# jeya-maria-jose/Medical-Transformer

Hardware: AMD Instinct MI355X
Metric: training images/sec (MedT, 3x128x128) (higher is better)
Workload: dtype f32; 1 GPU; MedT imgsize=128 bs=4/GPU train step (fwd+CE+bwd+Adam), BASELINE.json configs[2] (per GPU: also configs[3]'s shard); global_batch=4, parallelism=dp1

## Files before the change

### include/medt_abi.h

```cpp
#ifndef MEDT_ABI_H
#define MEDT_ABI_H

#include <stddef.h>
#include <stdint.h>

#ifdef __cplusplus
extern "C" {
#endif

#define MEDT_ABI_VERSION 11

#define MEDT_OK            0
#define MEDT_EINVAL       -1
#define MEDT_EUNSUPPORTED -2
#define MEDT_ELAUNCH      -3
#define MEDT_EWORKSPACE   -4

int         medt_abi_version(void);
const char* medt_last_error(void);

void*  medt_queue_create(void);
int    medt_queue_destroy(void* queue);
int    medt_queue_bind(void* queue, void* stream);
size_t medt_queue_pending(const void* queue);
int    medt_queue_flush(void* queue, void* stream);
int    medt_queue_flush2(void* queue, void* stream, void* aux_stream);
int    medt_queue_discard(void* queue);

typedef struct medt_axial_desc {
    int32_t N, C, H, W;
    int32_t G;
    int32_t axis;
    int32_t has_pos;
    int32_t stride;
    int32_t training;
    int32_t bn_groups;
    float   eps;
    float   momentum;
    int32_t out_relu;
    int32_t gate_mode;
    int32_t act_dtype;
} medt_axial_desc;

typedef struct medt_bn_ptrs {
    const float* weight;
    const float* bias;
    float*       running_mean;
    float*       running_var;
    int64_t*     num_batches_tracked;
} medt_bn_ptrs;

typedef struct medt_axial_params {
    const float* w_qkv;
    medt_bn_ptrs bn_qkv;
    medt_bn_ptrs bn_similarity;
    medt_bn_ptrs bn_output;
    const float* relative;
    const float* f_qr;
    const float* f_kr;
    const float* f_sve;
    const float* f_sv;
} medt_axial_params;

typedef struct medt_axial_saved {
    void*  qkv_raw;
    void*  stacked;
    float* lse;
    float* stats;
} medt_axial_saved;

typedef struct medt_axial_grads {
    float* w_qkv;
    float* bn_qkv_weight;  float* bn_qkv_bias;
    float* bn_sim_weight;  float* bn_sim_bias;
    float* bn_out_weight;  float* bn_out_bias;
    float* relative;
    float* gates;
} medt_axial_grads;

size_t medt_axial_stats_floats(const medt_axial_desc*);
size_t medt_axial_workspace_bytes(const medt_axial_desc*);

int medt_axial_layer_fwd(const medt_axial_desc*, const medt_axial_params*, const float* x, float* y,
                         const medt_axial_saved*, void* workspace, size_t workspace_bytes, void* stream);

int medt_axial_layer_bwd(const medt_axial_desc*, const medt_axial_params*, const float* x, const float* y,
                         const float* dy, const medt_axial_saved*, float* dx, const medt_axial_grads*,
                         void* workspace, size_t workspace_bytes, void* stream);

int medt_axial_core_stats(const medt_axial_desc*, const medt_axial_params*, const medt_axial_saved*,
                          void* workspace, size_t workspace_bytes, void* stream);
int medt_axial_core_fwd(const medt_axial_desc*, const medt_axial_params*, const medt_axial_saved*,
                        void* workspace, size_t workspace_bytes, void* stream);
int medt_axial_core_bwd(const medt_axial_desc*, const medt_axial_params*, const medt_axial_saved*, const float* dy,
                        void* workspace, size_t workspace_bytes, void* stream);

typedef struct medt_block_desc {
    int32_t N, C, width, H, W;
    int32_t G;
    int32_t training, bn_groups;
    float   eps, momentum;
} medt_block_desc;

typedef struct medt_block_params {
    const float*      w_down;
    medt_bn_ptrs      bn1;
    medt_axial_params height;
    medt_axial_params width;
    const float*      w_up;
    medt_bn_ptrs      bn2;
} medt_block_params;

typedef struct medt_block_saved {
    float* z1;
    float* y1;
    float* stats1;
    medt_axial_saved height;
    float* y_h;
    medt_axial_saved width;
    float* y_w;
    float* z2;
    float* stats2;
} medt_block_saved;

size_t medt_wopos_block_workspace_bytes(const medt_block_desc*);
int medt_wopos_block_fwd(const medt_block_desc*, const medt_block_params*, const float* x, float* y,
                         const medt_block_saved*, void* workspace, size_t workspace_bytes, void* stream);

typedef struct medt_block_s2_params {
    medt_block_params blk;
    const float*      w_ds;
    medt_bn_ptrs      bn_ds;
} medt_block_s2_params;
typedef struct medt_block_s2_saved {
    medt_block_saved blk;
    float *zd, *yd, *statsd;
} medt_block_s2_saved;
size_t medt_wopos_block_s2_workspace_bytes(const medt_block_desc*);
int medt_wopos_block_s2_fwd(const medt_block_desc*, const medt_block_s2_params*, const float* x, float* y,
                            const medt_block_s2_saved*, void* workspace, size_t workspace_bytes, void* stream);

typedef struct medt_block_grads {
    float *w_down, *bn1_weight, *bn1_bias;
    medt_axial_grads height, width;
    float *w_up, *bn2_weight, *bn2_bias;
} medt_block_grads;
size_t medt_wopos_block_bwd_workspace_bytes(const medt_block_desc*);
int medt_wopos_block_bwd(const medt_block_desc*, const medt_block_params*, const float* x, const float* y, const float* dy,
                         const medt_block_saved*, float* dx, const float* dx_add, const medt_block_grads*,
                         void* workspace, size_t workspace_bytes, void* stream);

typedef struct medt_conv_desc {
    int32_t N, Cin, H, W, Cout;
    int32_t K, stride, pad;
    int32_t has_bias;
    int32_t has_bn;
    int32_t has_res;
    int32_t relu;
    int32_t training, bn_groups;
    float   eps, momentum;
    int32_t lean;
} medt_conv_desc;

size_t medt_conv_stats_floats(const medt_conv_desc*);
size_t medt_conv_workspace_bytes(const medt_conv_desc*);

int medt_conv_block_fwd(const medt_conv_desc*, const float* x, const float* w, const float* bias,
                        const medt_bn_ptrs* bn, const float* res, float* z, float* y, float* stats,
                        void* workspace, size_t workspace_bytes, void* stream);
int medt_conv_block_bwd(const medt_conv_desc*, const float* x, const float* w, const medt_bn_ptrs* bn,
                        const float* z, const float* y, const float* stats, const float* dy,
                        float* dx, float* dw, float* dbias, float* dbn_weight, float* dbn_bias, float* dres,
                        const float* dx_add, void* workspace, size_t workspace_bytes, void* stream);

int medt_gate_mlp_fwd(const float* x, const float* w1, const float* b1, const float* w2, const float* b2, float* xn, float* h,
                      float* o, float* gates, int N, int C, int H, int W, int axis, void* stream);
int medt_gate_mlp_bwd(const float* dgates, const float* gates, const float* o, const float* h, const float* xn,
                      const float* w1, const float* w2, float* scratch, float* dw1, float* db1, float* dw2, float* db2,
                      float* dx, int N, int C, int H, int W, int axis, void* stream);

int medt_up2x_relu_add_fwd(const float* x, const float* skip, float* y, int NC, int H, int W, void* stream);
int medt_up2x_relu_bwd(const float* x, const float* dy, float* dx, int NC, int H, int W, void* stream);

int medt_patch_gather(const float* x, float* xp, int N, int C, int S, int P, int G, void* stream);
int medt_logo_merge_fwd(const float* x, const float* yp, float* y, int N, int C, int S, int P, int G, void* stream);
int medt_logo_merge_bwd(const float* dy, float* dx, float* dyp, int N, int C, int S, int P, int G, void* stream);

size_t medt_ce_partials(int N, int HW);
int medt_ce_fwd(const float* logits, const int64_t* target, float* partials, float* loss_out, int N, int K, int HW,
                int ignore_index, void* stream);
int medt_ce_bwd(const float* logits, const int64_t* target, const float* loss_out, const float* dloss, float* dlogits,
                int N, int K, int HW, int ignore_index, void* stream);

size_t medt_seg_loss_workspace(int N, int K, int HW);
size_t medt_seg_loss_out_floats(int N, int K);
int medt_seg_loss_fwd(const float* logits, const int64_t* target, const float* class_weight, float* partials, float* out,
                      int N, int K, int HW, int ignore_index, float ce_scale, float dice_scale, float eps, void* stream);
int medt_seg_loss_bwd(const float* logits, const int64_t* target, const float* class_weight, const float* out,
                      const float* dloss, float* dlogits, int N, int K, int HW, int ignore_index, float ce_scale,
                      float dice_scale, float eps, void* stream);

int medt_adam_step(float* p, const float* g, float* m, float* v, float* state, size_t n, float lr, float beta1,
                   float beta2, float eps, float weight_decay, float gscale, void* stream);

int medt_relu_mask(const float* a, const float* y, float* out, size_t n, void* stream);

int medt_seg_counts(const float* logits, const int64_t* target, int32_t* counts, int N, int K, int HW, float threshold,
                    void* stream);

int medt_window_gather(const float* image, float* windows, const int32_t* oy, const int32_t* ox, int C, int H, int W, int S,
                       int ny, int nx, void* stream);
int medt_window_blend(const float* win_logits, float* blended, uint8_t* mask, const int32_t* oy, const int32_t* ox, int K,
                      int H, int W, int S, int ny, int nx, float threshold, void* stream);

size_t medt_augment_param_floats(void);
size_t medt_augment_workspace(int N, int th, int tw);
int medt_augment_stats(const uint8_t* image, const float* params, float* workspace, int N, int H, int W, int C, int th,
                       int tw, void* stream);
int medt_augment_apply(const uint8_t* image, const uint8_t* mask, const float* params, float* workspace, float* out_image,
                       int64_t* out_mask, int N, int H, int W, int C, int th, int tw, int use_stats, void* stream);

#define MEDT_EDT_NONE    2147483647
#define MEDT_EDT_MAX_DIM 4096
int medt_edt_cols(const uint8_t* mask, int32_t* g2, int N, int H, int W, int border_mode, void* stream);
int medt_edt_rows(const int32_t* g2, const uint8_t* select, int32_t* d2, int N, int H, int W, void* stream);

int medt_signed_edt(const int64_t* target, int32_t* g2, int32_t* sd2, int N, int H, int W, int fg, int ignore_index, void* stream);
size_t medt_boundary_workspace(int N, int HW);
size_t medt_boundary_out_floats(int N);
int medt_boundary_fwd(const float* logits, const int64_t* target, const int32_t* sd2, const float* alpha, const float* base,
                      float* partials, float* out, int N, int K, int HW, int fg, int ignore_index, void* stream);
int medt_boundary_bwd(const float* logits, const int64_t* target, const int32_t* sd2, const float* out, const float* dloss,
                      float* dlogits, int N, int K, int HW, int fg, int ignore_index, int accumulate, void* stream);

int medt_object_edt2(const int32_t* labels, int32_t* scratch, int32_t* d1sq, int32_t* d2sq, int N, int H, int W, void* stream);
size_t medt_border_workspace(int N, int HW);
size_t medt_border_out_floats(int N);
int medt_border_fwd(const float* logits, const int64_t* target, const int32_t* d1sq, const int32_t* d2sq, float sigma,
                    const float* w0, const float* base, float* partials, float* out, int N, int K, int HW, int fg,
                    int ignore_index, void* stream);
int medt_border_bwd(const float* logits, const int64_t* target, const int32_t* d1sq, const int32_t* d2sq, float sigma,
                    const float* out, const float* dloss, float* dlogits, int N, int K, int HW, int fg, int ignore_index,
                    int accumulate, void* stream);

#define MEDT_LABEL_TILE_H  16
#define MEDT_LABEL_TILE_W  64
#define MEDT_LABEL_MAX_DIM 4096
size_t medt_label_workspace_bytes(int N, int H, int W);
int medt_label_components(const uint8_t* mask, int32_t* labels, int32_t* count, void* workspace, size_t workspace_bytes, int N,
                          int H, int W, int connectivity, int background, void* stream);
int medt_label_tables(const int32_t* labels, int32_t* area, uint8_t* frame, int N, int H, int W, int stride, int max_count,
                      void* stream);
int medt_label_select(const int32_t* labels, const uint8_t* keep, const uint8_t* mask, uint8_t* out, int N, int H, int W,
                      int stride, void* stream);

#define MEDT_PAIR_JOB_INTS 16
int medt_label_boxes(const int32_t* labels, int32_t* box, int N, int H, int W, int stride, int max_count, void* stream);
int medt_pair_hausdorff(const int32_t* la, const int32_t* lb, const int32_t* jobs, int32_t* scratch, int32_t* out, int n_jobs,
                        int col_blocks, int row_blocks, size_t scratch_elems, int n_out, int clear_out, int N, int H, int W,
                        void* stream);

#ifdef __cplusplus
}
#endif
#endif
```

### medical-transformer_amd/csrc/conv.hip

```cpp
#include "defer.h"
#include <type_traits>

namespace medt {

template <int K, int OT>
__global__ __launch_bounds__(MEDT_THREADS) void conv2d_fwd_kernel(
    const float* __restrict__ x, const float* __restrict__ w, const float* __restrict__ bias, float* __restrict__ y,
    float* __restrict__ partials, int Cin, int H, int W, int Cout, int Ho, int Wo, int stride, int pad, int relu,
    int npg, int y_bf16) {
    constexpr int KK = K * K;
    MEDT_STATIC_SHARED float red[MEDT_WAVES * OT * 2 * 2];
    const int HoWo = Ho * Wo, per_group = npg * HoWo, ppg = (per_group + MEDT_THREADS - 1) / MEDT_THREADS;
    const int grp = blockIdx.x / ppg, part = blockIdx.x - grp * ppg, o0 = blockIdx.y * OT;
    const int q = part * MEDT_THREADS + threadIdx.x;
    const bool ok = q < per_group;
    const int ni = ok ? q / HoWo : 0, p = ok ? q - ni * HoWo : 0;
    const int n = grp * npg + ni;
    const int ho = p / Wo, wo = p - ho * Wo;
    const int h0 = ho * stride - pad, w0 = wo * stride - pad;
    float acc[OT];
#pragma unroll
    for (int o = 0; o < OT; ++o) acc[o] = bias ? bias[o0 + o] : 0.f;
    const float* xn = x + (size_t)n * Cin * H * W;
    int off[KK];
#pragma unroll
    for (int kh = 0; kh < K; ++kh)
#pragma unroll
        for (int kw = 0; kw < K; ++kw) {
            const int h = h0 + kh, ww = w0 + kw;
            off[kh * K + kw] = (ok && (unsigned)h < (unsigned)H && (unsigned)ww < (unsigned)W) ? h * W + ww : -1;
        }
    const int HWi = H * W;
    constexpr int U = K == 1 ? 8 : (K == 3 ? 4 : 1);
    auto taps = [&](auto u_tag, int c) {
        constexpr int UU = decltype(u_tag)::value;
        float xr[UU][KK];
#pragma unroll
        for (int u = 0; u < UU; ++u)
#pragma unroll
            for (int t = 0; t < KK; ++t) xr[u][t] = xn[(size_t)(c + u) * HWi + max(off[t], 0)];
        MEDT_SCHED_FENCE();
#pragma unroll
        for (int u = 0; u < UU; ++u) {
            float xv[KK];
#pragma unroll
            for (int t = 0; t < KK; ++t) xv[t] = off[t] >= 0 ? xr[u][t] : 0.f;
#pragma unroll
            for (int o = 0; o < OT; ++o) {
                const float* wp = w + ((size_t)(o0 + o) * Cin + c + u) * KK;
#pragma unroll
                for (int t = 0; t < KK; ++t) acc[o] = fmaf(wp[t], xv[t], acc[o]);
            }
        }
        MEDT_SCHED_FENCE();
    };
    int c = 0;
    for (; c + U <= Cin; c += U) taps(std::integral_constant<int, U>{}, c);
    for (; c < Cin; ++c) taps(std::integral_constant<int, 1>{}, c);
    if (ok) {
        const size_t yo = ((size_t)n * Cout + o0) * HoWo + p;
#pragma unroll
        for (int o = 0; o < OT; ++o) st_act(y, yo + (size_t)o * HoWo, relu ? fmaxf(acc[o], 0.f) : acc[o], y_bf16);
    }
    if (partials) {
        float v[2 * OT];
#pragma unroll
        for (int o = 0; o < OT; ++o) {
            const float a = ok ? acc[o] : 0.f;
            v[2 * o] = a;
            v[2 * o + 1] = a * a;
        }
        block_sum_d<2 * OT>(v, red, reinterpret_cast<double*>(partials) + ((size_t)blockIdx.x * Cout + o0) * 2);
    }
}

int conv2d_parts_per_group(int N, int groups, int HoWo) { return cdiv((N / groups) * HoWo, MEDT_THREADS); }

static int pick_tile(int C, int max_tile, long position_blocks) {
    int t = max_tile;
    while (t > 1 && (C % t != 0 || position_blocks * (C / t) < 512)) t >>= 1;
    while (C % t != 0) t >>= 1;
    return t;
}

template <int K>
static int conv2d_fwd_k(const float* x, const float* w, const float* bias, float* y, float* partials, int N, int Cin,
                        int H, int W, int Cout, int Ho, int Wo, int stride, int pad, int relu, int groups,
                        hipStream_t s, int y_bf16) {
    const int npg = N / groups;
    const unsigned gx = (unsigned)(groups * conv2d_parts_per_group(N, groups, Ho * Wo));
#define MEDT_LAUNCH_FWD(OT)                                                                                        \
    hipLaunchKernelGGL((conv2d_fwd_kernel<K, OT>), dim3(gx, Cout / OT), dim3(MEDT_THREADS), 0, s, x, w, bias, y, partials, \
                       Cin, H, W, Cout, Ho, Wo, stride, pad, relu, npg, y_bf16)
    switch (pick_tile(Cout, K == 7 ? 8 : 16, gx)) {
        case 16: if constexpr (K != 7) { MEDT_LAUNCH_FWD(16); } break;
        case 8: MEDT_LAUNCH_FWD(8); break;
        case 4: MEDT_LAUNCH_FWD(4); break;
        case 2: MEDT_LAUNCH_FWD(2); break;
        default: MEDT_LAUNCH_FWD(1); break;
    }
#undef MEDT_LAUNCH_FWD
    return launch_status("conv2d_fwd");
}

static int conv_thin_mode() {
    static const int m = [] { const char* e = getenv("MEDT_CONV_THIN"); return e ? atoi(e) : 3; }();
    return m;
}
int conv_parts_per_group(int N, int groups, int HoWo, int Cin, int Cout, int K, int stride, int H, int W, int pad) {
    if (H > 0 && (conv_thin_mode() & 1) && !conv_use_mfma(Cin, Cout, K, stride, (long)N * HoWo) && conv_thin_ok(N, groups, Cin, H, W, Cout, K, stride, pad))
        return conv_thin_parts_per_group(N, groups, Cin, H, W, Cout, K, stride, pad);
    if (conv_fwd_ws_ok(Cin, Cout, K, stride, (long)N * HoWo)) return cdiv((N / groups) * HoWo, 64);
    if (!conv_use_mfma(Cin, Cout, K, stride, (long)N * HoWo)) return conv2d_parts_per_group(N, groups, HoWo);
    if (conv_mfma_scratch_floats(N, groups, HoWo, Cin, Cout, K, H > 0 && conv_rows16_ok(Cin, H, W, K, stride, pad)) > 0) return conv2d_parts_per_group(N, groups, HoWo);
    return conv_mfma_parts_per_group(N, groups, HoWo);
}

size_t conv2d_fwd_scratch_floats(int N, int groups, int Cin, int H, int W, int Cout, int K, int stride, int pad) {
    const int Ho = (H + 2 * pad - K) / stride + 1, Wo = (W + 2 * pad - K) / stride + 1;
    if (!conv_use_mfma(Cin, Cout, K, stride, (long)N * Ho * Wo)) return 0;
    return conv_mfma_scratch_floats(N, groups, Ho * Wo, Cin, Cout, K, conv_rows16_ok(Cin, H, W, K, stride, pad));
}

size_t conv2d_bwd_data_scratch_floats(int N, int Cin, int H, int W, int Cout, int K, int stride, int pad) {
    if (stride != 1 || K - 1 - pad < 0 || !conv_use_mfma(Cout, Cin, K, 1, (long)N * H * W)) return 0;
    return conv_mfma_scratch_floats(N, 1, H * W, Cout, Cin, K, conv_rows16_ok(Cout, H, W, K, 1, K - 1 - pad));
}

template <int K, int OT>
__global__ __launch_bounds__(MEDT_THREADS) void conv2d_fwd_ws_kernel(
    const float* __restrict__ x, const float* __restrict__ w, const float* __restrict__ bias, float* __restrict__ y,
    float* __restrict__ partials, int Cin, int H, int W, int Cout, int Ho, int Wo, int stride, int pad, int relu,
    int npg, int y_bf16) {
    constexpr int KK = K * K;
    MEDT_STATIC_SHARED float red[3][OT][64];
    extern __shared__ __attribute__((aligned(16))) float wl[];
    const int lane = threadIdx.x & 63, wv = __builtin_amdgcn_readfirstlane(threadIdx.x >> 6);
    const int HoWo = Ho * Wo, per_group = npg * HoWo, ppg = (per_group + 63) / 64;
    const int grp = blockIdx.x / ppg, part = blockIdx.x - grp * ppg, o0 = blockIdx.y * OT;
    {
        const int nw = OT * Cin * KK;
        const float* src = w + (size_t)o0 * Cin * KK;
        for (int e0 = threadIdx.x; e0 < nw; e0 += 8 * MEDT_THREADS) {
            float v[8];
#pragma unroll
            for (int u = 0; u < 8; ++u) v[u] = src[min(e0 + u * MEDT_THREADS, nw - 1)];
            MEDT_SCHED_FENCE();
#pragma unroll
            for (int u = 0; u < 8; ++u)
                if (e0 + u * MEDT_THREADS < nw) wl[e0 + u * MEDT_THREADS] = v[u];
        }
    }
    const int q = part * 64 + lane;
    const bool ok = q < per_group;
    const int ni = ok ? q / HoWo : 0, p = ok ? q - ni * HoWo : 0;
    const int n = grp * npg + ni;
    const int ho = p / Wo, wo = p - ho * Wo;
    const int h0 = ho * stride - pad, w0 = wo * stride - pad;
    int off[KK];
#pragma unroll
    for (int kh = 0; kh < K; ++kh)
#pragma unroll
        for (int kw = 0; kw < K; ++kw) {
            const int h = h0 + kh, ww = w0 + kw;
            off[kh * K + kw] = (ok && (unsigned)h < (unsigned)H && (unsigned)ww < (unsigned)W) ? h * W + ww : -1;
        }
    float acc[OT];
#pragma unroll
    for (int o = 0; o < OT; ++o) acc[o] = 0.f;
    const float* xn = x + (size_t)n * Cin * H * W;
    const int HWi = H * W;
    const int cb = (Cin * wv) / 4, ce = (Cin * (wv + 1)) / 4;
    __syncthreads();
    constexpr int U = K == 1 ? 16 : 4;
    auto taps = [&](auto u_tag, int c) {
        constexpr int UU = decltype(u_tag)::value;
        float xr[UU][KK];
#pragma unroll
        for (int u = 0; u < UU; ++u)
#pragma unroll
            for (int t = 0; t < KK; ++t) xr[u][t] = xn[(size_t)(c + u) * HWi + max(off[t], 0)];
        MEDT_SCHED_FENCE();
#pragma unroll
        for (int u = 0; u < UU; ++u) {
            float xv[KK];
#pragma unroll
            for (int t = 0; t < KK; ++t) xv[t] = off[t] >= 0 ? xr[u][t] : 0.f;
#pragma unroll
            for (int o = 0; o < OT; ++o) {
                const float* wp = wl + (o * Cin + c + u) * KK;
#pragma unroll
                for (int t = 0; t < KK; ++t) acc[o] = fmaf(wp[t], xv[t], acc[o]);
            }
        }
        MEDT_SCHED_FENCE();
    };
    int c = cb;
    for (; c + U <= ce; c += U) taps(std::integral_constant<int, U>{}, c);
    for (; c < ce; ++c) taps(std::integral_constant<int, 1>{}, c);
    if (wv > 0) {
#pragma unroll
        for (int o = 0; o < OT; ++o) red[wv - 1][o][lane] = acc[o];
    }
    __syncthreads();
    if (wv == 0) {
        const size_t yo = ((size_t)n * Cout + o0) * HoWo + p;
        double* pd = partials ? reinterpret_cast<double*>(partials) + ((size_t)blockIdx.x * Cout + o0) * 2 : nullptr;
#pragma unroll
        for (int o = 0; o < OT; ++o) {
            float v = acc[o] + (red[0][o][lane] + red[1][o][lane]) + red[2][o][lane];
            if (bias) v += bias[o0 + o];
            if (ok) st_act(y, yo + (size_t)o * HoWo, relu ? fmaxf(v, 0.f) : v, y_bf16);
            if (pd) {
                const float a = ok ? v : 0.f;
                const double s1 = wave_sum_d((double)a), s2 = wave_sum_d((double)(a * a));
                if (lane == 0) { pd[2 * o] = s1; pd[2 * o + 1] = s2; }
            }
        }
    }
}

static int conv_fwd_ws_tile(int Cin, int Cout, int K, long positions) {
    int ot = pick_tile(Cout, 8, (positions + 63) / 64);
    while (ot > 1 && (size_t)ot * Cin * K * K * sizeof(float) > 48 * 1024) ot >>= 1;
    return (size_t)ot * Cin * K * K * sizeof(float) <= 48 * 1024 ? ot : 0;
}

bool conv_fwd_ws_ok(int Cin, int Cout, int K, int stride, long positions) {
    static const bool on = true;
    return on && K == 3 && Cin * K * K >= 512 && positions <= 16384 && !conv_use_mfma(Cin, Cout, K, stride, positions) &&
           conv_fwd_ws_tile(Cin, Cout, K, positions) != 0;
}

static int conv2d_fwd_ws(const float* x, const float* w, const float* bias, float* y, float* partials, int N, int Cin, int H,
                         int W, int Cout, int Ho, int Wo, int stride, int pad, int relu, int groups, hipStream_t s,
                         int y_bf16) {
    const int npg = N / groups, ot = conv_fwd_ws_tile(Cin, Cout, 3, (long)N * Ho * Wo);
    const unsigned gx = (unsigned)(groups * cdiv(npg * Ho * Wo, 64));
    const size_t lds = (size_t)ot * Cin * 9 * sizeof(float);
#define MEDT_LAUNCH_FWS(OT)                                                                                            \
    hipLaunchKernelGGL((conv2d_fwd_ws_kernel<3, OT>), dim3(gx, Cout / OT), dim3(MEDT_THREADS), lds, s, x, w, bias, y, partials, \
                       Cin, H, W, Cout, Ho, Wo, stride, pad, relu, npg, y_bf16)
    switch (ot) {
        case 8: MEDT_LAUNCH_FWS(8); break;
        case 4: MEDT_LAUNCH_FWS(4); break;
        case 2: MEDT_LAUNCH_FWS(2); break;
        default: MEDT_LAUNCH_FWS(1); break;
    }
#undef MEDT_LAUNCH_FWS
    return launch_status("conv2d_fwd_ws");
}

int conv2d_fwd(const float* x, const float* w, const float* bias, float* y, float* partials, float* scratch, int N,
               int Cin, int H, int W, int Cout, int K, int stride, int pad, int relu, int groups, hipStream_t s,
               int y_bf16) {
    const int Ho = (H + 2 * pad - K) / stride + 1, Wo = (W + 2 * pad - K) / stride + 1;
    if (abl_skip(N >= 16 ? (K == 3 ? "conv3_fwd_l" : (K == 1 ? "conv1_fwd_l" : "conv7_fwd_l")) : (K == 3 ? "conv3_fwd_g" : (K == 1 ? "conv1_fwd_g" : "conv7_fwd_g")))) return MEDT_OK;
    if (!y_bf16 && conv_stem7_ok(Cin, H, W, Cout, K, stride, pad))
        return conv_stem7_fwd(x, w, bias, y, partials, N, H, W, Cout, relu, s);
    if (!y_bf16 && conv_use_mfma(Cin, Cout, K, stride, (long)N * Ho * Wo) &&
        (scratch || conv_mfma_scratch_floats(N, groups, Ho * Wo, Cin, Cout, K, conv_rows16_ok(Cin, H, W, K, stride, pad)) == 0))
        return conv_mfma_fwd(x, w, bias, y, partials, scratch, N, Cin, H, W, Cout, K, stride, pad, relu, groups, s);
    if (!y_bf16 && (conv_thin_mode() & 1) && !conv_use_mfma(Cin, Cout, K, stride, (long)N * Ho * Wo) && conv_thin_ok(N, groups, Cin, H, W, Cout, K, stride, pad))
        return conv_thin_fwd(x, w, bias, nullptr, y, partials, N, groups, Cin, H, W, Cout, relu, s);
    if (conv_fwd_ws_ok(Cin, Cout, K, stride, (long)N * Ho * Wo))
        return conv2d_fwd_ws(x, w, bias, y, partials, N, Cin, H, W, Cout, Ho, Wo, stride, pad, relu, groups, s, y_bf16);
    switch (K) {
        case 1: return conv2d_fwd_k<1>(x, w, bias, y, partials, N, Cin, H, W, Cout, Ho, Wo, stride, pad, relu, groups, s, y_bf16);
        case 3: return conv2d_fwd_k<3>(x, w, bias, y, partials, N, Cin, H, W, Cout, Ho, Wo, stride, pad, relu, groups, s, y_bf16);
        case 7: return conv2d_fwd_k<7>(x, w, bias, y, partials, N, Cin, H, W, Cout, Ho, Wo, stride, pad, relu, groups, s, y_bf16);
    }
    set_error("conv2d: kernel size %d unsupported (1, 3, 7)", K);
    return MEDT_EUNSUPPORTED;
}

template <int K, int CT>
__global__ __launch_bounds__(MEDT_THREADS) void conv2d_bwd_data_kernel(
    const float* __restrict__ dy, const float* __restrict__ w, float* __restrict__ dx, int N, int Cin, int H, int W,
    int Cout, int Ho, int Wo, int stride, int pad, const float* __restrict__ add) {
    constexpr int KK = K * K;
    const int HW = H * W;
    const long q = (long)blockIdx.x * MEDT_THREADS + threadIdx.x;
    const int c0 = blockIdx.y * CT;
    const bool ok = q < (long)N * HW;
    const int n = ok ? (int)(q / HW) : 0, p = ok ? (int)(q - (long)n * HW) : 0;
    const int h = p / W, ww = p - h * W;
    int off[KK];
#pragma unroll
    for (int kh = 0; kh < K; ++kh)
#pragma unroll
        for (int kw = 0; kw < K; ++kw) {
            const int hh = h + pad - kh, wq = ww + pad - kw;
            int o = -1;
            if (ok && hh >= 0 && wq >= 0 && hh % stride == 0 && wq % stride == 0) {
                const int ho = hh / stride, wo = wq / stride;
                if (ho < Ho && wo < Wo) o = ho * Wo + wo;
            }
            off[kh * K + kw] = o;
        }
    float acc[CT];
#pragma unroll
    for (int c = 0; c < CT; ++c) acc[c] = 0.f;
    const float* dyn = dy + (size_t)n * Cout * Ho * Wo;
    constexpr int U = K == 1 ? 8 : (K == 3 ? 4 : 1);
    const int HoWo = Ho * Wo;
    auto taps = [&](auto u_tag, int o) {
        constexpr int UU = decltype(u_tag)::value;
        float dr[UU][KK];
#pragma unroll
        for (int u = 0; u < UU; ++u)
#pragma unroll
            for (int t = 0; t < KK; ++t) dr[u][t] = dyn[(size_t)(o + u) * HoWo + max(off[t], 0)];
        MEDT_SCHED_FENCE();
#pragma unroll
        for (int u = 0; u < UU; ++u) {
            float dv[KK];
#pragma unroll
            for (int t = 0; t < KK; ++t) dv[t] = off[t] >= 0 ? dr[u][t] : 0.f;
#pragma unroll
            for (int c = 0; c < CT; ++c) {
                const float* wp = w + ((size_t)(o + u) * Cin + c0 + c) * KK;
#pragma unroll
                for (int t = 0; t < KK; ++t) acc[c] = fmaf(wp[t], dv[t], acc[c]);
            }
        }
        MEDT_SCHED_FENCE();
    };
    int o = 0;
    for (; o + U <= Cout; o += U) taps(std::integral_constant<int, U>{}, o);
    for (; o < Cout; ++o) taps(std::integral_constant<int, 1>{}, o);
    if (ok) {
        const size_t o0 = ((size_t)n * Cin + c0) * HW + p;
#pragma unroll
        for (int c = 0; c < CT; ++c) dx[o0 + (size_t)c * HW] = add ? acc[c] + add[o0 + (size_t)c * HW] : acc[c];
    }
}

template <int K, int CT, int TM = (1 << (K * K)) - 1>
__global__ __launch_bounds__(MEDT_THREADS) void conv2d_bwd_data_ws_kernel(
    const float* __restrict__ dy, const float* __restrict__ w, float* __restrict__ dx, int N, int Cin, int H, int W,
    int Cout, int Ho, int Wo, int stride, int pad, const float* __restrict__ add, int stage_dy) {
    constexpr int KK = K * K;
    MEDT_STATIC_SHARED float red[3][CT][64];
    extern __shared__ __attribute__((aligned(16))) float wl[];
    const int lane = threadIdx.x & 63, wv = threadIdx.x >> 6;
    const int HW = H * W;
    const long q = (long)blockIdx.x * 64 + lane;
    const int c0 = blockIdx.y * CT;
    if constexpr (TM == (1 << KK) - 1) {
        const int nw = Cout * CT * KK;
        for (int e0 = threadIdx.x; e0 < nw; e0 += 8 * MEDT_THREADS) {
            float v[8];
#pragma unroll
            for (int u = 0; u < 8; ++u) {
                const int e = min(e0 + u * MEDT_THREADS, nw - 1), o = e / (CT * KK), r = e - o * (CT * KK);
                v[u] = w[((size_t)o * Cin + c0) * KK + r];
            }
            MEDT_SCHED_FENCE();
#pragma unroll
            for (int u = 0; u < 8; ++u)
                if (e0 + u * MEDT_THREADS < nw) wl[e0 + u * MEDT_THREADS] = v[u];
        }
    } else {
        constexpr int NL = __builtin_popcount((unsigned)TM);
        const int nw = Cout * CT * NL;
        for (int e0 = threadIdx.x; e0 < nw; e0 += 8 * MEDT_THREADS) {
            float v[8];
            int dst[8];
#pragma unroll
            for (int u = 0; u < 8; ++u) {
                const int e = min(e0 + u * MEDT_THREADS, nw - 1), oc = e / NL, tl = e - oc * NL;
                int t = 0, seen = 0;
#pragma unroll
                for (int b = 0; b < KK; ++b)
                    if ((TM >> b) & 1) { if (seen == tl) t = b; ++seen; }
                const int o = oc / CT, c = oc - o * CT;
                dst[u] = oc * KK + t;
                v[u] = w[((size_t)o * Cin + c0 + c) * KK + t];
            }
            MEDT_SCHED_FENCE();
#pragma unroll
            for (int u = 0; u < 8; ++u)
                if (e0 + u * MEDT_THREADS < nw) wl[dst[u]] = v[u];
        }
    }
    float* dl = wl + Cout * CT * KK;
    const int HoWo_ = Ho * Wo;
    const int nb0 = (int)(((long)blockIdx.x * 64) / HW);
    const int img_stride = Cout * HoWo_ + 1;
    if (stage_dy) {
        const int nb1 = min(N - 1, (int)(((long)blockIdx.x * 64 + 63) / HW));
        const int per = Cout * HoWo_, cnt = (nb1 - nb0 + 1) * per;
        const float* src = dy + (size_t)nb0 * per;
        for (int e0 = threadIdx.x; e0 < cnt; e0 += 8 * MEDT_THREADS) {
            float v[8];
#pragma unroll
            for (int u = 0; u < 8; ++u) v[u] = src[min(e0 + u * MEDT_THREADS, cnt - 1)];
            MEDT_SCHED_FENCE();
#pragma unroll
            for (int u = 0; u < 8; ++u) {
                const int e = e0 + u * MEDT_THREADS;
                if (e < cnt) { const int im = e / per; dl[im * img_stride + (e - im * per)] = v[u]; }
            }
        }
    }
    const bool ok = q < (long)N * HW;
    const int n = ok ? (int)(q / HW) : 0, p = ok ? (int)(q - (long)n * HW) : 0;
    const int h = p / W, ww = p - h * W;
    int off[KK];
#pragma unroll
    for (int kh = 0; kh < K; ++kh)
#pragma unroll
        for (int kw = 0; kw < K; ++kw) {
            const int hh = h + pad - kh, wq = ww + pad - kw;
            int o = -1;
            if (ok && hh >= 0 && wq >= 0 && hh % stride == 0 && wq % stride == 0) {
                const int ho = hh / stride, wo = wq / stride;
                if (ho < Ho && wo < Wo) o = ho * Wo + wo;
            }
            off[kh * K + kw] = o;
        }
    float acc[CT];
#pragma unroll
    for (int c = 0; c < CT; ++c) acc[c] = 0.f;
    const float* dyn = dy + (size_t)n * Cout * Ho * Wo;
    const int ob = (Cout * wv) / 4, oe = (Cout * (wv + 1)) / 4;
// ... 431 lines not shown
```

### medical-transformer_amd/csrc/conv_small.hip

```cpp
#include "medt_common.h"
#include "medt_kernels.h"
#include <stdlib.h>
#include <type_traits>

namespace medt {

struct SmallConvArgs {
    const float *x, *w, *res;
    medt_bn_ptrs bn;
    float *z, *y, *partials;
    int N, Cin, H, W, Cout, stride, npg, relu, training;
    float eps;
};

__device__ __forceinline__ void conv_small_scale_shift(double s, double ss, double count, const medt_bn_ptrs& bn, int ch,
                                                       float eps, int training, float& scale, float& shift) {
    const float g = bn.weight[ch], b = bn.bias[ch];
    if (training) {
        const double mean = s / count;
        double var = ss / count - mean * mean;
        if (var < 0.0) var = 0.0;
        const double rstd = 1.0 / sqrt(var + (double)eps);
        scale = (float)(g * rstd);
        shift = (float)(b - mean * g * rstd);
    } else {
        const float mean = bn.running_mean[ch];
        const float rstd = (float)(1.0 / sqrt((double)bn.running_var[ch] + (double)eps));
        scale = g * rstd;
        shift = b - mean * g * rstd;
    }
}

__device__ __forceinline__ void conv_small_scale_shift_p(double s, double ss, double count, const float* prm, float eps,
                                                         int training, float& scale, float& shift) {
    const float g = prm[0], b = prm[1];
    if (training) {
        const double mean = s / count;
        double var = ss / count - mean * mean;
        if (var < 0.0) var = 0.0;
        const double rstd = 1.0 / sqrt(var + (double)eps);
        scale = (float)(g * rstd);
        shift = (float)(b - mean * g * rstd);
    } else {
        const float mean = prm[2];
        const float rstd = (float)(1.0 / sqrt((double)prm[3] + (double)eps));
        scale = g * rstd;
        shift = b - mean * g * rstd;
    }
}

constexpr int SC_NOC_MAX = 16;

static __host__ __device__ inline int conv_small_threads(int P) { return P <= 256 ? 256 : (P <= 512 ? 512 : 1024); }
static __host__ __device__ inline int conv_small_ksplit(int P, int Cin) {
    int ks = 1;
    const int T = conv_small_threads(P);
    while (ks * 2 <= 16 && ks * 2 * P <= T && Cin % (ks * 2 * 8) == 0) ks *= 2;
    return ks;
}

template <int T, int SC_NOC>
__global__ __launch_bounds__(T) void conv1x1_bn_small_fwd_kernel(SmallConvArgs a) {
    extern __shared__ __attribute__((aligned(16))) float smem[];
    const int grp = blockIdx.x, oc0 = blockIdx.y * SC_NOC, tid = threadIdx.x, lane = tid & 63, wave = tid >> 6;
    constexpr int NW = T >> 6;
    const int Cin = a.Cin, W = a.W, HW = a.H * a.W, st = a.stride, Ho = a.H / st, Wo = a.W / st, HoWo = Ho * Wo;
    const int P = a.npg * HoWo, n0 = grp * a.npg;
    const int KS = conv_small_ksplit(P, Cin), cpk = Cin / KS;
    float* Z = smem;
    float* Wl = Z + SC_NOC * P;
    float* sc = Wl + Cin * SC_NOC;
    float* sh = sc + SC_NOC;
    float* prm = sh + SC_NOC;
    float* sums = prm + 4 * SC_NOC;
    float* Zp = sums + 2 * SC_NOC;
    if (tid < SC_NOC) {
        const int ch = oc0 + tid;
        prm[tid * 4] = a.bn.weight[ch];
        prm[tid * 4 + 1] = a.bn.bias[ch];
        if (!a.training) {
            prm[tid * 4 + 2] = a.bn.running_mean[ch];
            prm[tid * 4 + 3] = a.bn.running_var[ch];
        }
    }
    const bool act = tid < P * KS;
    const int ks = act ? tid / P : 0, q = act ? tid - ks * P : 0, ni = q / HoWo, po = q - ni * HoWo;
    const int ho = po / Wo, wo = po - ho * Wo;
    const float* xp = a.x + ((size_t)(n0 + ni) * Cin + (size_t)ks * cpk) * HW + (ho * st) * W + wo * st;
    constexpr int WB = 8, XB = T == 1024 ? 16 : 32;
    const int nW = SC_NOC * Cin;
    float wr[WB], xv[XB];
    auto load_w = [&](int base) {
#pragma unroll
        for (int k = 0; k < WB; ++k) {
            const int e = min(base + tid + k * T, nW - 1), oc = e / Cin;
            wr[k] = a.w[(size_t)(oc0 + oc) * Cin + (e - oc * Cin)];
        }
    };
    auto store_w = [&](int base) {
#pragma unroll
        for (int k = 0; k < WB; ++k) {
            const int e = base + tid + k * T;
            if (e < nW) { const int oc = e / Cin; Wl[(e - oc * Cin) * SC_NOC + oc] = wr[k]; }
        }
    };
    auto load_x = [&](int c0) {
        if constexpr (T == 1024) {
#pragma unroll
            for (int k = 0; k < XB; ++k) xv[k] = xp[(size_t)min(c0 + k, cpk - 1) * HW];
        } else {
#pragma unroll
            for (int k8 = 0; k8 < XB; k8 += 8)
                if (c0 + k8 < cpk) {
#pragma unroll
                    for (int k = k8; k < k8 + 8; ++k) xv[k] = xp[(size_t)(c0 + k) * HW];
                }
        }
    };
    load_w(0);
    load_x(0);
    MEDT_SCHED_FENCE();
    store_w(0);
    for (int base = WB * T; base < nW; base += WB * T) {
        load_w(base);
        MEDT_SCHED_FENCE();
        store_w(base);
    }
    __syncthreads();
    float acc[SC_NOC];
#pragma unroll
    for (int o = 0; o < SC_NOC; ++o) acc[o] = 0.f;
    for (int c0 = 0; c0 < cpk; c0 += XB) {
        if (c0) {
            load_x(c0);
            MEDT_SCHED_FENCE();
        }
#pragma unroll
        for (int k8 = 0; k8 < XB; k8 += 8)
            if (c0 + k8 < cpk) {
#pragma unroll
                for (int k = k8; k < k8 + 8; ++k) {
                    const float* wrow = Wl + (ks * cpk + c0 + k) * SC_NOC;
#pragma unroll
                    for (int o = 0; o < SC_NOC; o += 4) {
                        const float4 w4 = *reinterpret_cast<const float4*>(wrow + o);
                        acc[o] = fmaf(w4.x, xv[k], acc[o]);
                        acc[o + 1] = fmaf(w4.y, xv[k], acc[o + 1]);
                        acc[o + 2] = fmaf(w4.z, xv[k], acc[o + 2]);
                        acc[o + 3] = fmaf(w4.w, xv[k], acc[o + 3]);
                    }
                }
            }
    }
    if (KS == 1) {
        if (act) {
#pragma unroll
            for (int o = 0; o < SC_NOC; ++o) {
                Z[o * P + q] = acc[o];
                a.z[((size_t)(n0 + ni) * a.Cout + oc0 + o) * HoWo + po] = acc[o];
            }
        }
    } else {
        if (act) {
#pragma unroll
            for (int o = 0; o < SC_NOC; ++o) Zp[(ks * SC_NOC + o) * P + q] = acc[o];
        }
        __syncthreads();
        for (int item = tid; item < SC_NOC * P; item += T) {
            const int oc = item / P, qq = item - oc * P, n2 = qq / HoWo, p2 = qq - n2 * HoWo;
            float v = Zp[item];
            for (int k = 1; k < KS; ++k) v += Zp[k * SC_NOC * P + item];
            Z[item] = v;
            a.z[((size_t)(n0 + n2) * a.Cout + oc0 + oc) * HoWo + p2] = v;
        }
    }
    constexpr int RI = 16;
    float rv[RI];
    if (a.res) {
#pragma unroll
        for (int k = 0; k < RI; ++k) {
            const int item = min(tid + k * T, SC_NOC * P - 1);
            const int oc = item / P, qq = item - oc * P, n2 = qq / HoWo, p2 = qq - n2 * HoWo;
            rv[k] = a.res[((size_t)(n0 + n2) * a.Cout + oc0 + oc) * HoWo + p2];
        }
    }
    __syncthreads();
    for (int oc = wave; oc < SC_NOC; oc += NW) {
        float s = 0.f, ss = 0.f;
        for (int qq = lane; qq < P; qq += 64) s += Z[oc * P + qq];
        s = wave_sum(s);
        const float m = s * (1.f / (float)P);
        for (int qq = lane; qq < P; qq += 64) {
            const float dv = Z[oc * P + qq] - m;
            ss = fmaf(dv, dv, ss);
        }
        ss = wave_sum(ss);
        if (lane == 0) {
            sums[oc * 2] = s;
            sums[oc * 2 + 1] = ss;
        }
    }
    __syncthreads();
    if (tid < SC_NOC) {
        const int ch = oc0 + tid;
        double s, ss;
        centered_to_raw(sums[tid * 2], sums[tid * 2 + 1], sums[tid * 2] * (1.f / (float)P), (double)P, s, ss);
        conv_small_scale_shift_p(s, ss, (double)P, prm + tid * 4, a.eps, a.training, sc[tid], sh[tid]);
        if (a.training) {
            double* dp = reinterpret_cast<double*>(a.partials) + ((size_t)grp * a.Cout + ch) * 2;
            dp[0] = s;
            dp[1] = ss;
        }
    }
    __syncthreads();
#pragma unroll
    for (int k = 0; k < RI; ++k) {
        const int item = tid + k * T;
        if (item < SC_NOC * P) {
            const int oc = item / P, qq = item - oc * P, n2 = qq / HoWo, p2 = qq - n2 * HoWo;
            const size_t idx = ((size_t)(n0 + n2) * a.Cout + oc0 + oc) * HoWo + p2;
            float v = fmaf(Z[item], sc[oc], sh[oc]);
            if (a.res) v += rv[k];
            if (a.relu) v = fmaxf(v, 0.f);
            a.y[idx] = v;
        }
    }
}

static size_t conv_small_lds(int P, int Cin, int noc) {
    const int ks = conv_small_ksplit(P, Cin);
    return ((size_t)noc * P + (size_t)Cin * noc + 8 * noc + (ks > 1 ? (size_t)ks * noc * P : 0)) * sizeof(float);
}

static int conv_small_noc(int P, int Cin) {
    static const int min_noc = 16;
    for (int noc = SC_NOC_MAX; noc >= min_noc; noc >>= 1)
        if (conv_small_lds(P, Cin, noc) <= 64 * 1024) return noc;
    return 0;
}

static bool conv_small_enabled() {
    static const bool on = [] { const char* e = getenv("MEDT_DISABLE_SMALL"); return !(e && e[0] == '1'); }();
    return on;
}

bool conv_small_ok(const medt_conv_desc& d) {
    if (!conv_small_enabled() || !d.has_bn || d.K != 1 || d.pad != 0 || d.has_bias) return false;
    if (d.stride < 1 || d.H % d.stride || d.W % d.stride) return false;
    if ((d.Cin & 15) || (d.Cout % SC_NOC_MAX)) return false;
    const int P = (d.N / d.bn_groups) * (d.H / d.stride) * (d.W / d.stride);
    if (!(P <= 1024 && conv_small_noc(P, d.Cin) != 0)) return false;
#ifndef MEDT_AB_SMALL_ANYGRID
    if (d.bn_groups == 1 && d.Cout / conv_small_noc(P, d.Cin) < 32) return false;
#endif
    return true;
}

int conv_small_fwd(const medt_conv_desc& d, const float* x, const float* w, const medt_bn_ptrs& bn, const float* res,
                   float* z, float* y, float* partials, hipStream_t s) {
    if (abl_skip("conv_small_fwd")) return MEDT_OK;
    SmallConvArgs a;
    a.x = x; a.w = w; a.res = d.has_res ? res : nullptr; a.bn = bn; a.z = z; a.y = y; a.partials = partials;
    a.N = d.N; a.Cin = d.Cin; a.H = d.H; a.W = d.W; a.Cout = d.Cout; a.stride = d.stride; a.npg = d.N / d.bn_groups;
    a.relu = d.relu; a.training = d.training ? 1 : 0; a.eps = d.eps;
    const int P = a.npg * (d.H / d.stride) * (d.W / d.stride);
    const int threads = conv_small_threads(P);
    const int noc = conv_small_noc(P, d.Cin);
    const dim3 grid(d.bn_groups, d.Cout / noc);
    const size_t lds = conv_small_lds(P, d.Cin, noc);
#define MEDT_SMALL_CONV(TT)                                                                              \
    do {                                                                                                 \
        if (noc == 16) hipLaunchKernelGGL((conv1x1_bn_small_fwd_kernel<TT, 16>), grid, dim3(TT), lds, s, a); \
        else hipLaunchKernelGGL((conv1x1_bn_small_fwd_kernel<TT, 8>), grid, dim3(TT), lds, s, a);         \
    } while (0)
    if (threads == 256) MEDT_SMALL_CONV(256);
    else if (threads == 512) MEDT_SMALL_CONV(512);
    else MEDT_SMALL_CONV(1024);
#undef MEDT_SMALL_CONV
    return launch_status("conv1x1_bn_small_fwd");
}

struct SmallBnBwdArgs {
    const float *dy, *y, *z, *weight;
    BnStats st;
    float *g, *dz, *partials;
    int C, HW, npg, relu, training;
};

__global__ __launch_bounds__(MEDT_THREADS) void bn_act_bwd_small_kernel(SmallBnBwdArgs a) {
    const int grp = blockIdx.x, c = blockIdx.y * MEDT_WAVES + (threadIdx.x >> 6), lane = threadIdx.x & 63;
    if (c >= a.C) return;
    const int HW = a.HW, P = a.npg * HW, gc = grp * a.C + c;
    const float mean = a.st.mean[gc], rstd = a.st.rstd[gc];
    float s1 = 0.f, s2 = 0.f;
    for (int q = lane; q < P; q += 64) {
        const int ni = q / HW, p = q - ni * HW;
        const size_t idx = ((size_t)(grp * a.npg + ni) * a.C + c) * HW + p;
        float d = a.dy[idx];
        if (a.relu && !(a.y[idx] > 0.f)) d = 0.f;
        if (a.g) a.g[idx] = d;
        s1 += d;
        s2 = fmaf(d, (a.z[idx] - mean) * rstd, s2);
    }
    s1 = wave_sum(s1);
    s2 = wave_sum(s2);
    if (lane == 0) {
        a.partials[(size_t)gc * 2] = s1;
        a.partials[(size_t)gc * 2 + 1] = s2;
    }
    const double A = (double)a.weight[c] * (double)rstd;
    float c0 = (float)A, c1 = 0.f, c2 = 0.f;
    if (a.training) {
        const double m1 = (double)s1 / (double)P, m2 = (double)s2 / (double)P;
        c1 = (float)(-A * (double)rstd * m2);
        c2 = (float)(A * ((double)rstd * (double)mean * m2 - m1));
    }
    for (int q = lane; q < P; q += 64) {
        const int ni = q / HW, p = q - ni * HW;
        const size_t idx = ((size_t)(grp * a.npg + ni) * a.C + c) * HW + p;
        float d = a.dy[idx];
        if (a.relu && !(a.y[idx] > 0.f)) d = 0.f;
        a.dz[idx] = fmaf(c0, d, fmaf(c1, a.z[idx], c2));
    }
}

template <int TT, int NK = 4>
__global__ __launch_bounds__(TT) void bn_act_bwd_chan_kernel(SmallBnBwdArgs a) {
    MEDT_STATIC_SHARED float red[2 * (TT / 64)];
    const int grp = blockIdx.x, c = blockIdx.y, tid = threadIdx.x;
    const int HW = a.HW, P = a.npg * HW, gc = grp * a.C + c;
    const float mean = a.st.mean[gc], rstd = a.st.rstd[gc];
    float4 dv[NK], zv[NK];
    size_t at[NK];
    float s1 = 0.f, s2 = 0.f;
#pragma unroll
    for (int k = 0; k < NK; ++k) {
        const int q = 4 * (tid + k * TT);
        dv[k] = make_float4(0.f, 0.f, 0.f, 0.f);
        zv[k] = dv[k];
        at[k] = 0;
        if (q < P) {
            const int ni = q / HW, p = q - ni * HW;
            const size_t idx = ((size_t)(grp * a.npg + ni) * a.C + c) * HW + p;
            at[k] = idx;
            float4 d = *reinterpret_cast<const float4*>(a.dy + idx);
            if (a.relu) {
                const float4 yv = *reinterpret_cast<const float4*>(a.y + idx);
                if (!(yv.x > 0.f)) d.x = 0.f;
                if (!(yv.y > 0.f)) d.y = 0.f;
                if (!(yv.z > 0.f)) d.z = 0.f;
                if (!(yv.w > 0.f)) d.w = 0.f;
            }
            if (a.g) *reinterpret_cast<float4*>(a.g + idx) = d;
            const float4 zz = *reinterpret_cast<const float4*>(a.z + idx);
            dv[k] = d;
            zv[k] = zz;
            s1 += (d.x + d.y) + (d.z + d.w);
            s2 = fmaf(d.x, (zz.x - mean) * rstd, s2);
            s2 = fmaf(d.y, (zz.y - mean) * rstd, s2);
            s2 = fmaf(d.z, (zz.z - mean) * rstd, s2);
            s2 = fmaf(d.w, (zz.w - mean) * rstd, s2);
        }
    }
    s1 = wave_sum(s1);
    s2 = wave_sum(s2);
    if ((tid & 63) == 0) { red[(tid >> 6) * 2] = s1; red[(tid >> 6) * 2 + 1] = s2; }
    __syncthreads();
    s1 = 0.f;
    s2 = 0.f;
#pragma unroll
    for (int w = 0; w < TT / 64; ++w) { s1 += red[w * 2]; s2 += red[w * 2 + 1]; }
    if (tid == 0) {
        a.partials[(size_t)gc * 2] = s1;
        a.partials[(size_t)gc * 2 + 1] = s2;
    }
    const double A = (double)a.weight[c] * (double)rstd;
    float c0 = (float)A, c1 = 0.f, c2 = 0.f;
    if (a.training) {
        const double m1 = (double)s1 / (double)P, m2 = (double)s2 / (double)P;
        c1 = (float)(-A * (double)rstd * m2);
        c2 = (float)(A * ((double)rstd * (double)mean * m2 - m1));
    }
#pragma unroll
    for (int k = 0; k < NK; ++k) {
        const int q = 4 * (tid + k * TT);
        if (q < P) {
            float4 o;
            o.x = fmaf(c0, dv[k].x, fmaf(c1, zv[k].x, c2));
            o.y = fmaf(c0, dv[k].y, fmaf(c1, zv[k].y, c2));
            o.z = fmaf(c0, dv[k].z, fmaf(c1, zv[k].z, c2));
            o.w = fmaf(c0, dv[k].w, fmaf(c1, zv[k].w, c2));
            *reinterpret_cast<float4*>(a.dz + at[k]) = o;
        }
    }
}

int bn_chan_threads(const medt_conv_desc& d, int HoWo) {
#ifdef MEDT_AB_BN_CHAN_16K
    static const int pmax = 16384;
#else
    static const int pmax = 32768;
#endif
    if (!d.has_bn || (HoWo & 3)) return 0;
    const long P = (long)(d.N / d.bn_groups) * HoWo;
    if (P > pmax) return 0;
    return P <= 4096 ? 256 : 1024;
}

int bn_act_bwd_chan(const medt_conv_desc& d, const float* dy, const float* y, const float* z, BnStats st,
                    const float* weight, float* g, float* dz, float* partials, int HoWo, hipStream_t s) {
    SmallBnBwdArgs a;
    a.dy = dy; a.y = y; a.z = z; a.weight = weight; a.st = st; a.g = g; a.dz = dz; a.partials = partials;
    a.C = d.Cout; a.HW = HoWo; a.npg = d.N / d.bn_groups; a.relu = d.relu; a.training = d.training ? 1 : 0;
    const dim3 grid(d.bn_groups, d.Cout);
    if (bn_chan_threads(d, HoWo) == 256) hipLaunchKernelGGL(bn_act_bwd_chan_kernel<256>, grid, dim3(256), 0, s, a);
    else if ((long)a.npg * HoWo <= 16384) hipLaunchKernelGGL(bn_act_bwd_chan_kernel<1024>, grid, dim3(1024), 0, s, a);
    else hipLaunchKernelGGL((bn_act_bwd_chan_kernel<1024, 8>), grid, dim3(1024), 0, s, a);
    return launch_status("bn_act_bwd_chan");
// ... 226 lines not shown
```

### medical-transformer_amd/csrc/elementwise.hip

```cpp
#include "medt_kernels.h"
#include <stdint.h>
#include <stdlib.h>

namespace medt {

static inline unsigned grid1d(size_t total) { return (unsigned)((total + MEDT_THREADS - 1) / MEDT_THREADS); }

__global__ __launch_bounds__(MEDT_THREADS) void bn_apply_act_kernel(const float* __restrict__ z, BnStats st,
                                                                    const float* __restrict__ res,
                                                                    float* __restrict__ y, int C, int HW, int npg,
                                                                    int relu, size_t total) {
    const size_t idx = (size_t)blockIdx.x * MEDT_THREADS + threadIdx.x;
    if (idx >= total) return;
    const size_t nc = idx / HW;
    const int c = (int)(nc % C), n = (int)(nc / C);
    const int gc = (n / npg) * C + c;
    float v = fmaf(z[idx], st.scale[gc], st.shift[gc]);
    if (res) v += res[idx];
    if (relu) v = fmaxf(v, 0.f);
    y[idx] = v;
}

int bn_apply_act(const float* z, BnStats st, const float* res, float* y, int N, int C, int HW, int groups, int relu,
                 hipStream_t s) {
    const size_t total = (size_t)N * C * HW;
    hipLaunchKernelGGL(bn_apply_act_kernel, dim3(grid1d(total)), dim3(MEDT_THREADS), 0, s, z, st, res, y, C, HW,
                       N / groups, relu, total);
    return launch_status("bn_apply_act");
}

struct BnFinApplyArgs {
    const float *z, *partials, *weight, *bias, *running_mean, *running_var, *res;
    float* y;
    BnStats st;
    int C, HW, npg, ppg, parts, relu, training, vec4;
    double count;
    float eps;
};
constexpr int BFA_PER_THREAD = 16;
__global__ __launch_bounds__(MEDT_THREADS) void bn_fin_apply_kernel(BnFinApplyArgs a) {
    MEDT_STATIC_SHARED double redd[2 * MEDT_WAVES];
    const int grp = blockIdx.x / a.parts, part = blockIdx.x - grp * a.parts, c = blockIdx.y, tid = threadIdx.x;
    const int gc = grp * a.C + c;
    const float gam = a.weight[c], bet = a.bias[c];
    float mean_f, rstd_f, scale, shift;
    if (a.training) {
        const double* pd = reinterpret_cast<const double*>(a.partials);
        double s = 0.0, ss = 0.0;
        for (int p = tid; p < a.ppg; p += MEDT_THREADS) {
            const double* q = pd + ((size_t)(grp * a.ppg + p) * a.C + c) * 2;
            s += q[0];
            ss += q[1];
        }
        s = wave_sum_d(s);
        ss = wave_sum_d(ss);
        if ((tid & 63) == 0) { redd[(tid >> 6) * 2] = s; redd[(tid >> 6) * 2 + 1] = ss; }
        __syncthreads();
        s = 0.0;
        ss = 0.0;
#pragma unroll
        for (int w = 0; w < MEDT_WAVES; ++w) { s += redd[w * 2]; ss += redd[w * 2 + 1]; }
        const double mean = s / a.count;
        double var = ss / a.count - mean * mean;
        if (var < 0.0) var = 0.0;
        const double rstd = 1.0 / sqrt(var + (double)a.eps);
        mean_f = (float)mean;
        rstd_f = (float)rstd;
        scale = (float)(gam * rstd);
        shift = (float)(bet - mean * gam * rstd);
    } else {
        mean_f = a.running_mean[c];
        rstd_f = (float)(1.0 / sqrt((double)a.running_var[c] + (double)a.eps));
        scale = gam * rstd_f;
        shift = bet - mean_f * gam * rstd_f;
    }
    if (part == 0 && tid == 0) {
        a.st.mean[gc] = mean_f;
        a.st.rstd[gc] = rstd_f;
        a.st.scale[gc] = scale;
        a.st.shift[gc] = shift;
    }
    const int HW = a.HW, P = a.npg * HW;
    const int q0 = part * (MEDT_THREADS * BFA_PER_THREAD);
    const int q1 = q0 + MEDT_THREADS * BFA_PER_THREAD < P ? q0 + MEDT_THREADS * BFA_PER_THREAD : P;
    if (a.vec4) {
        for (int q = q0 + 4 * tid; q < q1; q += 4 * MEDT_THREADS) {
            const int ni = q / HW, p = q - ni * HW;
            const size_t idx = ((size_t)(grp * a.npg + ni) * a.C + c) * HW + p;
            const float4 zz = *reinterpret_cast<const float4*>(a.z + idx);
            float4 v;
            v.x = fmaf(zz.x, scale, shift);
            v.y = fmaf(zz.y, scale, shift);
            v.z = fmaf(zz.z, scale, shift);
            v.w = fmaf(zz.w, scale, shift);
            if (a.res) {
                const float4 r = *reinterpret_cast<const float4*>(a.res + idx);
                v.x += r.x; v.y += r.y; v.z += r.z; v.w += r.w;
            }
            if (a.relu) { v.x = fmaxf(v.x, 0.f); v.y = fmaxf(v.y, 0.f); v.z = fmaxf(v.z, 0.f); v.w = fmaxf(v.w, 0.f); }
            *reinterpret_cast<float4*>(a.y + idx) = v;
        }
    } else {
        for (int q = q0 + tid; q < q1; q += MEDT_THREADS) {
            const int ni = q / HW, p = q - ni * HW;
            const size_t idx = ((size_t)(grp * a.npg + ni) * a.C + c) * HW + p;
            float v = fmaf(a.z[idx], scale, shift);
            if (a.res) v += a.res[idx];
            if (a.relu) v = fmaxf(v, 0.f);
            a.y[idx] = v;
        }
    }
}

int bn_fin_apply(const float* z, const float* partials, int ppg, double count, const medt_bn_ptrs& bn, float eps, int training,
                 BnStats st, const float* res, float* y, int N, int C, int HW, int groups, int relu, hipStream_t s) {
    BnFinApplyArgs a;
    a.z = z; a.partials = partials; a.weight = bn.weight; a.bias = bn.bias; a.running_mean = bn.running_mean;
    a.running_var = bn.running_var; a.res = res; a.y = y; a.st = st; a.C = C; a.HW = HW; a.npg = N / groups; a.ppg = ppg;
    a.parts = cdiv(a.npg * HW, MEDT_THREADS * BFA_PER_THREAD); a.relu = relu; a.training = training; a.count = count;
    a.vec4 = ((HW & 3) == 0 && (((uintptr_t)z | (uintptr_t)y | (uintptr_t)res) & 15) == 0) ? 1 : 0;
    a.eps = eps;
    hipLaunchKernelGGL(bn_fin_apply_kernel, dim3(groups * a.parts, C), dim3(MEDT_THREADS), 0, s, a);
    return launch_status("bn_fin_apply");
}

__global__ __launch_bounds__(MEDT_THREADS) void bn_act_bwd_stats_kernel(const float* __restrict__ dy,
                                                                        const float* __restrict__ y,
                                                                        const float* __restrict__ z, BnStats st,
                                                                        float* __restrict__ g,
                                                                        float* __restrict__ partials, int C, int HW,
                                                                        int npg, int relu) {
    MEDT_STATIC_SHARED float red[MEDT_WAVES * 2];
    const int per_group = npg * HW, ppg = (per_group + MEDT_THREADS - 1) / MEDT_THREADS;
    const int grp = blockIdx.x / ppg, part = blockIdx.x - grp * ppg, c = blockIdx.y;
    const int q = part * MEDT_THREADS + threadIdx.x;
    float v[2] = {0.f, 0.f};
    if (q < per_group) {
        const int ni = q / HW, p = q - ni * HW;
        const int gc = grp * C + c;
        const size_t idx = ((size_t)(grp * npg + ni) * C + c) * HW + p;
        float d = dy[idx];
        if (relu && !(y[idx] > 0.f)) d = 0.f;
        if (g) g[idx] = d;
        v[0] = d;
        v[1] = d * ((z[idx] - st.mean[gc]) * st.rstd[gc]);
    }
    block_sum<2>(v, red, partials + ((size_t)blockIdx.x * C + c) * 2);
}

int bn_act_bwd_stats(const float* dy, const float* y, const float* z, BnStats st, float* g, float* partials, int N, int C,
                     int HW, int groups, int relu, hipStream_t s) {
    const int ppg = cdiv((N / groups) * HW, MEDT_THREADS);
    hipLaunchKernelGGL(bn_act_bwd_stats_kernel, dim3(groups * ppg, C), dim3(MEDT_THREADS), 0, s, dy, y, z, st, g,
                       partials, C, HW, N / groups, relu);
    return launch_status("bn_act_bwd_stats");
}

__global__ __launch_bounds__(MEDT_THREADS) void bn_bwd_apply_kernel(const float* __restrict__ g,
                                                                    const float* __restrict__ z,
                                                                    const float* __restrict__ coef,
                                                                    float* __restrict__ dz, int C, int HW, int npg,
                                                                    size_t total) {
    const size_t idx = (size_t)blockIdx.x * MEDT_THREADS + threadIdx.x;
    if (idx >= total) return;
    const size_t nc = idx / HW;
    const int c = (int)(nc % C), n = (int)(nc / C);
    const float* cf = coef + ((size_t)(n / npg) * C + c) * 3;
    dz[idx] = fmaf(cf[0], g[idx], fmaf(cf[1], z[idx], cf[2]));
}

int bn_bwd_apply(const float* g, const float* z, const float* coef, float* dz, int N, int C, int HW, int groups,
                 hipStream_t s) {
    const size_t total = (size_t)N * C * HW;
    hipLaunchKernelGGL(bn_bwd_apply_kernel, dim3(grid1d(total)), dim3(MEDT_THREADS), 0, s, g, z, coef, dz, C, HW,
                       N / groups, total);
    return launch_status("bn_bwd_apply");
}

__global__ __launch_bounds__(MEDT_THREADS) void relu_mask_kernel(const float* __restrict__ a, const float* __restrict__ y,
                                                                 float* __restrict__ out, size_t total) {
    const size_t i = (size_t)blockIdx.x * MEDT_THREADS + threadIdx.x;
    if (i < total) out[i] = y[i] > 0.f ? a[i] : 0.f;
}

int relu_mask(const float* a, const float* y, float* out, size_t total, hipStream_t s) {
    hipLaunchKernelGGL(relu_mask_kernel, dim3(grid1d(total)), dim3(MEDT_THREADS), 0, s, a, y, out, total);
    return launch_status("relu_mask");
}

__global__ __launch_bounds__(MEDT_THREADS) void relu_kernel(const float* __restrict__ x, float* __restrict__ y,
                                                            size_t total) {
    const size_t i = (size_t)blockIdx.x * MEDT_THREADS + threadIdx.x;
    if (i < total) y[i] = fmaxf(x[i], 0.f);
}

int relu_fwd(const float* x, float* y, size_t total, hipStream_t s) {
    hipLaunchKernelGGL(relu_kernel, dim3(grid1d(total)), dim3(MEDT_THREADS), 0, s, x, y, total);
    return launch_status("relu");
}

struct Lerp { int i0, i1; float l; };
__device__ __forceinline__ Lerp src_index(int o, int n_in) {
    float s = 0.5f * ((float)o + 0.5f) - 0.5f;
    if (s < 0.f) s = 0.f;
    Lerp r;
    r.i0 = (int)s;
    r.i1 = r.i0 + (r.i0 < n_in - 1 ? 1 : 0);
    r.l = s - (float)r.i0;
    return r;
}

__device__ __forceinline__ float up_value(float v00, float v01, float v10, float v11, float lh, float lw) {
    const float h0 = 1.f - lh, w0 = 1.f - lw;
    const float t0 = fmaf(lw, v01, w0 * v00), t1 = fmaf(lw, v11, w0 * v10);
    return fmaf(lh, t1, h0 * t0);
}

__device__ __forceinline__ float up_sample(const float* __restrict__ xp, int H, int W, int ho, int wo) {
    const Lerp a = src_index(ho, H), b = src_index(wo, W);
    return up_value(xp[a.i0 * W + b.i0], xp[a.i0 * W + b.i1], xp[a.i1 * W + b.i0], xp[a.i1 * W + b.i1], a.l, b.l);
}

__global__ __launch_bounds__(MEDT_THREADS) void up2x_relu_add_kernel(const float* __restrict__ x,
                                                                     const float* __restrict__ skip,
                                                                     float* __restrict__ y, int H, int W, size_t total) {
    const size_t idx = (size_t)blockIdx.x * MEDT_THREADS + threadIdx.x;
    if (idx >= total) return;
    const int Wo = 2 * W, Ho = 2 * H;
    const int wo = (int)(idx % Wo), ho = (int)((idx / Wo) % Ho);
    const size_t nc = idx / ((size_t)Wo * Ho);
    float v = fmaxf(up_sample(x + nc * H * W, H, W, ho, wo), 0.f);
    if (skip) v += skip[idx];
    y[idx] = v;
}

__global__ __launch_bounds__(MEDT_THREADS) void up2x_relu_add4_kernel(const float* __restrict__ x,
                                                                      const float* __restrict__ skip,
                                                                      float* __restrict__ y, int H, int W, size_t total4) {
    const size_t idx = (size_t)blockIdx.x * MEDT_THREADS + threadIdx.x;
    if (idx >= total4) return;
    const int Wq = W / 2, Ho = 2 * H;
    const int t = (int)(idx % Wq), ho = (int)((idx / Wq) % Ho);
    const size_t nc = idx / ((size_t)Wq * Ho);
    const float* xp = x + nc * H * W;
    const Lerp a = src_index(ho, H);
    const int cc[4] = {max(2 * t - 1, 0), 2 * t, 2 * t + 1, min(2 * t + 2, W - 1)};
    float r0[4], r1[4];
#pragma unroll
    for (int k = 0; k < 4; ++k) {
        r0[k] = xp[a.i0 * W + cc[k]];
        r1[k] = xp[a.i1 * W + cc[k]];
    }
    constexpr int C0[4] = {0, 1, 1, 2};
    float v[4];
#pragma unroll
    for (int k = 0; k < 4; ++k) {
        const Lerp b = src_index(4 * t + k, W);
        v[k] = fmaxf(up_value(r0[C0[k]], r0[C0[k] + 1], r1[C0[k]], r1[C0[k] + 1], a.l, b.l), 0.f);
    }
    const size_t o = (nc * Ho + ho) * (size_t)(2 * W) + 4 * t;
    if (skip) {
        const float4 sk = *reinterpret_cast<const float4*>(skip + o);
        v[0] += sk.x; v[1] += sk.y; v[2] += sk.z; v[3] += sk.w;
    }
    *reinterpret_cast<float4*>(y + o) = make_float4(v[0], v[1], v[2], v[3]);
}

int up2x_relu_add_fwd(const float* x, const float* skip, float* y, int NC, int H, int W, hipStream_t s) {
    const size_t total = (size_t)NC * 4 * H * W;
    static const bool vec = true;
    if (vec && (W & 1) == 0 && ((uintptr_t)y & 15) == 0 && (!skip || ((uintptr_t)skip & 15) == 0)) {
        hipLaunchKernelGGL(up2x_relu_add4_kernel, dim3(grid1d(total / 4)), dim3(MEDT_THREADS), 0, s, x, skip, y, H, W, total / 4);
        return launch_status("up2x_relu_add4");
    }
    hipLaunchKernelGGL(up2x_relu_add_kernel, dim3(grid1d(total)), dim3(MEDT_THREADS), 0, s, x, skip, y, H, W, total);
    return launch_status("up2x_relu_add");
// ... 1661 lines not shown
```

### medical-transformer_amd/csrc/medt_api.hip

```cpp
#include "defer.h"
#include "fin_inline.h"
#include <string.h>

namespace medt {

static thread_local char g_err[512] = "";

void set_error(const char* fmt, ...) {
    va_list ap;
    va_start(ap, fmt);
    vsnprintf(g_err, sizeof(g_err), fmt, ap);
    va_end(ap);
}

bool abl_skip(const char* family) {
#ifndef MEDT_ABLATE
    (void)family;
    return false;
#else
    static const char* env = [] {
        const char* e = getenv("MEDT_SKIP");
        if (e && *e)
            fprintf(stderr, "libmedt_hip: MEDT_SKIP=%s -- TIMING EXPERIMENT: these kernel families are NOT launched, every result of "
                            "this process is garbage\n", e);
// ... 336 lines not shown
        return conv2d_bwd_weight(w.dqkv, qkv_raw, w.coef_qkv, x, gr->w_qkv, w.dw_scratch, g.N, g.C, g.H, g.W, 2 * g.C,
                                 1, 1, 0, g.groups, s, queue_for(s));
    }
    const float* ymask = nullptr;
    if (d->out_relu) {
#ifndef MEDT_AB_NO_MASK_FUSE
        if (w.sweep) ymask = y;
#endif
        if (!ymask) {
            if ((rc = relu_mask(dy, y, w.dy_masked, (size_t)g.N * g.C * (g.H / d->stride) * (g.W / d->stride), s))) return rc;
            dy = w.dy_masked;
        }
    }
    const float out_dscale = 1.f / (float)(d->stride * d->stride);
    const bool sim_inl = w.sweep && g.pos && inline_fin_ok(tr, g.groups, w.plan.nparts) &&
                         axial_out_bwd_stats_tables_ok(*d, sim_tables_blocks(g), g.L);
    const TablesJob btj{p->relative, w.tables, g.hq, g.L, sim_tables_blocks(g)};
    if ((rc = axial_out_bwd_stats(*d, stacked, dy, st.out, w.part_ob, s, sim_inl ? &btj : nullptr, ymask))) return rc;
    BfinSrc ob = no_bfin_src();
    if (w.sweep && inline_fin_ok(tr, g.groups, ppg)) {
        ob.j = BfinJob{w.part_ob, ppg, g.groups, g.OC, tr, g.row_count, out_dscale, st.out, p->bn_output.weight, w.coef_out,
                       gr->bn_out_weight, gr->bn_out_bias};
        ob.on = 1;
    } else if ((rc = bn_bwd_finalize(w.part_ob, ppg, g.groups, g.OC, g.row_count, out_dscale, st.out, p->bn_output.weight, tr,
                                     w.coef_out, gr->bn_out_weight, gr->bn_out_bias, s))) return rc;
    BfinSrc qb = no_bfin_src();
    if (w.sweep && (!g.bf16 || w.raw32) && inline_fin_ok(tr, g.groups, w.qb_rpg)) {
        qb.j = BfinJob{w.part_qb, w.qb_rpg, g.groups, 2 * g.C, tr, g.row_count, 1.f, st.qkv, p->bn_qkv.weight, w.coef_qkv,
                       gr->bn_qkv_weight, gr->bn_qkv_bias};
        qb.on = 1;
    }
    if ((rc = attention_core_bwd(g, d, p, w, qkv_raw, stacked, sv->lse, dy, st, gates, gr->gates != nullptr,
                                 gr->bn_sim_weight, gr->bn_sim_bias, s, ob.on ? &ob : nullptr, sim_inl, qb.on ? &qb : nullptr, ymask))) return rc;
    const float *bq_raw = qkv_raw, *bq_coef = w.coef_qkv;
    static const bool bf16_fused = true;
    if (g.bf16 && w.raw32) {
        if (!qb.on && (rc = bn_bwd_finalize(w.part_qb, w.qb_rpg, g.groups, 2 * g.C, g.row_count, 1.f, st.qkv, p->bn_qkv.weight, tr,
                                         w.coef_qkv, gr->bn_qkv_weight, gr->bn_qkv_bias, s))) return rc;
        bq_raw = w.raw32;
    } else if (g.bf16 && bf16_fused && (long)g.N * 2 * g.C <= 65535) {
        if ((rc = bn_bwd_fin_apply_bf16(w.part_qb, w.qb_rpg, g.groups, 2 * g.C, g.row_count, 1.f, st.qkv, p->bn_qkv.weight, tr,
                                        w.coef_qkv, gr->bn_qkv_weight, gr->bn_qkv_bias, w.dqkv, qkv_raw, g.N, g.HW, s))) return rc;
        bq_raw = nullptr;
        bq_coef = nullptr;
    } else {
        if (!qb.on && (rc = bn_bwd_finalize(w.part_qb, w.qb_rpg, g.groups, 2 * g.C, g.row_count, 1.f, st.qkv, p->bn_qkv.weight, tr,
                                            w.coef_qkv, gr->bn_qkv_weight, gr->bn_qkv_bias, s))) return rc;
        if (g.bf16) {
            if ((rc = bn_bwd_apply_raw_bf16(w.dqkv, qkv_raw, w.coef_qkv, g.N, 2 * g.C, g.HW, g.groups, s))) return rc;
            bq_raw = nullptr;
            bq_coef = nullptr;
        }
    }
    if ((rc = conv1x1_bwd_data(w.dqkv, bq_raw, bq_coef, p->w_qkv, dx, g.N, g.C, 2 * g.C, g.HW, g.groups, s)))
        return rc;
    Queue* q = queue_for(s);
    if ((rc = conv2d_bwd_weight(w.dqkv, bq_raw, bq_coef, x, gr->w_qkv, w.dw_scratch, g.N, g.C, g.H, g.W, 2 * g.C, 1,
                                1, 0, g.groups, s, q))) return rc;
    if (g.pos) {
        const int rel_rows = w.sweep ? (int)w.sweep_blocks + g.groups * g.G : (int)w.nblocks;
        const float* gate_src = w.sweep ? w.gate_rows : w.gate_part;
        const int gate_rows = w.sweep ? g.groups * g.G : (int)w.nblocks;
        if (q) q->reduce.push_back(RJob{w.rel_part, gr->relative, rel_rows, 2 * g.gp * TL});
        else if ((rc = reduce_rows(w.rel_part, rel_rows, 2 * g.gp * TL, gr->relative, s))) return rc;
        if (gr->gates && d->gate_mode == 2) {
            if ((rc = gate_seq_reduce(w.gate_part, gr->gates, g.groups * g.spg, g.G, s))) return rc;
        } else if (gr->gates) {
            const bool sig = d->gate_mode == 1 && p->f_qr;
            if (q && !sig) q->reduce.push_back(RJob{gate_src, gr->gates, gate_rows, 4});
            else {
                if ((rc = reduce_rows(gate_src, gate_rows, 4, sig ? w.gate_tmp : gr->gates, s))) return rc;
                if (sig && (rc = gate_sigmoid_bwd(w.gate_tmp, w.gate_eff, gr->gates, s))) return rc;
            }
        }
    }
    return MEDT_OK;
}


}

namespace medt {
struct ConvGeom { int Ho, Wo, HoWo, ppg, ppg_bwd, splits; size_t out_elems; };
static int conv_geom(const medt_conv_desc* d, ConvGeom* g) {
    if (!d || d->N <= 0 || d->Cin <= 0 || d->Cout <= 0 || d->H <= 0 || d->W <= 0 || d->stride < 1 || d->pad < 0) {
        set_error("conv: bad descriptor"); return MEDT_EINVAL;
    }
    if (d->K != 1 && d->K != 3 && d->K != 7) { set_error("conv: kernel size %d unsupported (1, 3, 7)", d->K); return MEDT_EUNSUPPORTED; }
    if (d->has_bn && (d->bn_groups < 1 || d->N % d->bn_groups)) { set_error("conv: bad bn_groups"); return MEDT_EINVAL; }
    if (d->has_bn && d->has_bias) { set_error("conv: bias followed by BatchNorm is not on the reference's path"); return MEDT_EUNSUPPORTED; }
    if (!d->has_bn && d->has_res) { set_error("conv: residual without BatchNorm is not on the reference's path"); return MEDT_EUNSUPPORTED; }
    g->Ho = (d->H + 2 * d->pad - d->K) / d->stride + 1;
    g->Wo = (d->W + 2 * d->pad - d->K) / d->stride + 1;
    if (g->Ho <= 0 || g->Wo <= 0) { set_error("conv: empty output"); return MEDT_EINVAL; }
    if ((double)d->N * d->Cin * d->H * d->W >= 2147483648.0 || (double)d->N * d->Cout * g->Ho * g->Wo >= 2147483648.0 ||
        (double)d->Cout * d->Cin * d->K * d->K >= 2147483648.0) {
        set_error("conv: tensors of 2^31 elements and more are unsupported"); return MEDT_EUNSUPPORTED;
    }
    g->HoWo = g->Ho * g->Wo;
    g->ppg = conv_stem7_ok(d->Cin, d->H, d->W, d->Cout, d->K, d->stride, d->pad)
                 ? conv_stem7_parts_per_group(d->N, d->has_bn ? d->bn_groups : 1, g->HoWo)
                 : conv_parts_per_group(d->N, d->has_bn ? d->bn_groups : 1, g->HoWo, d->Cin, d->Cout, d->K, d->stride, d->H, d->W, d->pad);
    g->ppg_bwd = conv2d_parts_per_group(d->N, d->has_bn ? d->bn_groups : 1, g->HoWo);
    g->splits = conv2d_bwd_weight_splits(d->N, d->Cin, d->Cout, d->K, g->Ho, g->Wo);
    g->out_elems = (size_t)d->N * d->Cout * g->HoWo;
    return MEDT_OK;
}
struct ConvWs {
    float *partials, *coef, *bias_scratch, *gbuf, *dz, *dw_scratch, *wt, *ksplit, *ksplit_fwd, *ksplit_bwd;
    ConvWs(Carver& c, const medt_conv_desc* d, const ConvGeom& g) {
        wt = c.take<float>((size_t)d->Cout * d->Cin * d->K * d->K);
        const size_t kf = conv2d_fwd_scratch_floats(d->N, d->has_bn ? d->bn_groups : 1, d->Cin, d->H, d->W, d->Cout, d->K,
                                                    d->stride, d->pad);
        const size_t kb = conv2d_bwd_data_scratch_floats(d->N, d->Cin, d->H, d->W, d->Cout, d->K, d->stride, d->pad);
        ksplit = c.take<float>(kf > kb ? kf : kb);
        if (!(kf > 0 || kb > 0)) ksplit = nullptr;
        ksplit_fwd = kf > 0 ? ksplit : nullptr;
        ksplit_bwd = kb > 0 ? ksplit : nullptr;
        partials = c.take<float>(d->has_bn ? (size_t)d->bn_groups * (2 * g.ppg > g.ppg_bwd ? 2 * g.ppg : g.ppg_bwd) * d->Cout * 2 : 0);
        coef = c.take<float>(d->has_bn ? (size_t)d->bn_groups * d->Cout * 3 : 0);
        bias_scratch = c.take<float>((size_t)16 * d->Cout);
        gbuf = c.take<float>(g.out_elems);
        dz = c.take<float>(d->has_bn ? g.out_elems : 0);
        dw_scratch = c.take<float>((size_t)g.splits * d->Cout * d->Cin * d->K * d->K);
    }
};
}

extern "C" {

static bool conv_preflip(const medt_conv_desc* d) {
    static const bool on = true;
    return on && d->training && d->K == 3 && conv2d_bwd_data_flips(d->N, d->Cin, d->H, d->W, d->Cout, d->K, d->stride, d->pad);
}
static size_t conv_bn_stats_floats(const medt_conv_desc* d) { return d->has_bn ? (size_t)4 * d->bn_groups * d->Cout : 0; }
static float* conv_preflip_ptr(const medt_conv_desc* d, float* stats) { return stats + align_up(conv_bn_stats_floats(d), 64); }

size_t medt_conv_stats_floats(const medt_conv_desc* d) {
    if (!d) return 0;
    const size_t bn = (d->has_bn && d->bn_groups > 0 && d->Cout > 0) ? (size_t)4 * d->bn_groups * d->Cout : 0;
    ConvGeom g;
    if (conv_geom(d, &g)) return bn;
    return conv_preflip(d) ? align_up(bn, 64) + (size_t)d->Cout * d->Cin * d->K * d->K : bn;
}

size_t medt_conv_workspace_bytes(const medt_conv_desc* d) {
    ConvGeom g;
    if (conv_geom(d, &g)) return 0;
    Carver c(nullptr, 0);
    ConvWs w(c, d, g);
    return align_up(c.off, 256) + 256;
}

int medt_conv_block_fwd(const medt_conv_desc* d, const float* x, const float* w, const float* bias,
                        const medt_bn_ptrs* bn, const float* res, float* z, float* y, float* stats, void* ws,
                        size_t ws_bytes, void* stream) {
    ConvGeom g;
    int rc = conv_geom(d, &g);
    if (rc) return rc;
    if (!x || !w || !y || (d->has_bias && !bias) || (d->has_bn && (!bn || !z || !stats)) || (d->has_res && !res)) {
        set_error("conv fwd: null pointer"); return MEDT_EINVAL;
    }
    hipStream_t s = (hipStream_t)stream;
    Carver c(ws, ws_bytes);
    ConvWs cw(c, d, g);
    if (!ws || !c.ok()) { set_error("conv workspace too small: need %zu", c.off); return MEDT_EWORKSPACE; }
    if (stats && conv_preflip(d)) {
        float* wt = conv_preflip_ptr(d, stats);
        if (Queue* q = queue_for(s)) q->flip.push_back(FlipJob{w, wt, d->Cout, d->Cin, d->K});
        else if ((rc = conv_flip_weights(w, wt, d->Cout, d->Cin, d->K, s))) return rc;
    }
    if (!d->has_bn)
        return conv2d_fwd(x, w, d->has_bias ? bias : nullptr, y, nullptr, cw.ksplit_fwd, d->N, d->Cin, d->H, d->W, d->Cout,
                          d->K, d->stride, d->pad, d->relu, 1, s);
    const int tr = d->training ? 1 : 0;
    if (!tr && (!bn->running_mean || !bn->running_var)) { set_error("conv fwd: eval mode needs running statistics"); return MEDT_EINVAL; }
    if (tr && (double)(d->N / d->bn_groups) * g.HoWo <= 1.0) {
        set_error("conv fwd: training-mode BatchNorm needs more than 1 value per channel"); return MEDT_EINVAL;
    }
    BnStats st(stats, d->bn_groups * d->Cout);
    if (conv_small_ok(*d)) {
        if ((rc = conv_small_fwd(*d, x, w, *bn, res, z, y, cw.partials, s))) return rc;
        if (Queue* q = queue_for(s)) {
            q->fin.push_back(FinJob{make_fin(cw.partials, 1, d->Cout, (double)(d->N / d->bn_groups) * g.HoWo, *bn, st),
                                    d->bn_groups, tr, d->momentum, d->eps});
            return MEDT_OK;
        }
        return bn_finalize(cw.partials, 1, d->bn_groups, d->Cout, (double)(d->N / d->bn_groups) * g.HoWo, *bn, d->momentum,
                           d->eps, tr, st, s);
    }
    if ((rc = conv2d_fwd(x, w, nullptr, z, tr ? cw.partials : nullptr, cw.ksplit_fwd, d->N, d->Cin, d->H, d->W, d->Cout, d->K,
                         d->stride, d->pad, 0, d->bn_groups, s))) return rc;
    static const bool fused_fin = true;
    const double count = (double)(d->N / d->bn_groups) * g.HoWo;
    if (!fused_fin) {
        if ((rc = bn_finalize(cw.partials, g.ppg, d->bn_groups, d->Cout, count, *bn, d->momentum, d->eps, tr, st, s))) return rc;
        return bn_apply_act(z, st, d->has_res ? res : nullptr, y, d->N, d->Cout, g.HoWo, d->bn_groups, d->relu, s);
    }
    if ((rc = bn_fin_apply(z, cw.partials, g.ppg, count, *bn, d->eps, tr, st, d->has_res ? res : nullptr, y, d->N, d->Cout,
                           g.HoWo, d->bn_groups, d->relu, s))) return rc;
    if (!tr) return MEDT_OK;
    if (Queue* q = queue_for(s)) {
        q->fin.push_back(FinJob{make_fin(cw.partials, g.ppg, d->Cout, count, *bn, st), d->bn_groups, 2, d->momentum, d->eps});
        return MEDT_OK;
    }
    return bn_finalize(cw.partials, g.ppg, d->bn_groups, d->Cout, count, *bn, d->momentum, d->eps, 2, st, s);
}

int medt_conv_block_bwd(const medt_conv_desc* d, const float* x, const float* w, const medt_bn_ptrs* bn, const float* z,
                        const float* y, const float* stats, const float* dy, float* dx, float* dw, float* dbias,
                        float* dbn_weight, float* dbn_bias, float* dres, const float* dx_add, void* ws, size_t ws_bytes,
                        void* stream) {
    ConvGeom g;
    int rc = conv_geom(d, &g);
    if (rc) return rc;
    if (!x || !w || !dy || !dw || (d->relu && !y) || (d->has_bn && (!bn || !z || !stats || !dbn_weight || !dbn_bias)) ||
        (d->has_bias && !dbias)) { set_error("conv bwd: null pointer"); return MEDT_EINVAL; }
    Carver c(ws, ws_bytes);
    ConvWs cw(c, d, g);
    if (!ws || !c.ok()) { set_error("conv workspace too small: need %zu", c.off); return MEDT_EWORKSPACE; }
    hipStream_t s = (hipStream_t)stream;
    const float* grad_out;
    bool dx_done = false;
    if (d->has_bn) {
        BnStats st(const_cast<float*>(stats), d->bn_groups * d->Cout);
        float* gb = (d->has_res && dres) ? dres : cw.gbuf;
        const bool small = conv_small_ok(*d);
        const bool aligned = ((((uintptr_t)dy | (uintptr_t)y | (uintptr_t)z | (uintptr_t)dres | (uintptr_t)cw.dz) & 15) == 0);
        if (small || (aligned && bn_chan_threads(*d, g.HoWo))) {
            if (small && dx && aligned && !d->lean && bn_dgrad1x1_small_ok(*d)) {
                rc = bn_dgrad1x1_small(*d, dy, y, z, st, bn->weight, w, dx_add, (d->has_res && dres) ? dres : nullptr,
                                       cw.dz, cw.partials, dx, s);
                dx_done = true;
            } else if (small)
                rc = bn_act_bwd_small(*d, dy, y, z, st, bn->weight, (d->has_res && dres) ? dres : nullptr, cw.dz,
                                      cw.partials, g.HoWo, s);
            else
                rc = bn_act_bwd_chan(*d, dy, y, z, st, bn->weight, (d->has_res && dres) ? dres : nullptr, cw.dz,
                                     cw.partials, g.HoWo, s);
            if (rc) return rc;
            if (Queue* q = queue_for(s))
                q->bfin.push_back(BfinJob{cw.partials, 1, d->bn_groups, d->Cout, d->training ? 1 : 0,
                                          (double)(d->N / d->bn_groups) * g.HoWo, 1.f, st, bn->weight, cw.coef, dbn_weight,
                                          dbn_bias});
            else if ((rc = bn_bwd_finalize(cw.partials, 1, d->bn_groups, d->Cout, (double)(d->N / d->bn_groups) * g.HoWo, 1.f,
                                           st, bn->weight, d->training ? 1 : 0, cw.coef, dbn_weight, dbn_bias, s))) return rc;
        } else {
        if ((rc = bn_act_bwd_stats(dy, y, z, st, gb, cw.partials, d->N, d->Cout, g.HoWo, d->bn_groups, d->relu, s))) return rc;
        if ((rc = bn_bwd_finalize(cw.partials, g.ppg_bwd, d->bn_groups, d->Cout,
                                  (double)(d->N / d->bn_groups) * g.HoWo, 1.f, st, bn->weight, d->training ? 1 : 0, cw.coef,
                                  dbn_weight, dbn_bias, s))) return rc;
        if ((rc = bn_bwd_apply(gb, z, cw.coef, cw.dz, d->N, d->Cout, g.HoWo, d->bn_groups, s))) return rc;
        }
        grad_out = cw.dz;
    } else if (d->relu) {
        if ((rc = relu_mask(dy, y, cw.gbuf, g.out_elems, s))) return rc;
        grad_out = cw.gbuf;
    } else {
        grad_out = dy;
    }
    const bool preflipped = stats && conv_preflip(d);
    if (dx && !dx_done && (rc = conv2d_bwd_data(grad_out, w, dx, preflipped ? conv_preflip_ptr(d, const_cast<float*>(stats)) : cw.wt, cw.ksplit_bwd,
                                                d->N, d->Cin, d->H, d->W, d->Cout, d->K, d->stride, d->pad, s, dx_add, preflipped))) return rc;
    Queue* q = queue_for(s);
    if (d->has_bias) {
        if (q) {
            const int splits = channel_sum_splits_for(d->N, g.HoWo);
            q->csum.push_back(CJob{grad_out, splits == 1 ? dbias : cw.bias_scratch, d->N, d->Cout, g.HoWo, splits});
            if (splits > 1) q->reduce.push_back(RJob{cw.bias_scratch, dbias, splits, d->Cout});
        } else if ((rc = channel_sum(grad_out, dbias, cw.bias_scratch, d->N, d->Cout, g.HoWo, s))) return rc;
    }
    return conv2d_bwd_weight(grad_out, nullptr, nullptr, x, dw, cw.dw_scratch, d->N, d->Cin, d->H, d->W, d->Cout, d->K, d->stride,
                             d->pad, 1, s, q);
}

size_t medt_wopos_block_workspace_bytes(const medt_block_desc* d) {
    if (!d || !wopos_block_ok(*d)) return 0;
    return align_up(wopos_block_part_doubles(*d) * sizeof(double), 256) + 256;
}

int medt_wopos_block_fwd(const medt_block_desc* d, const medt_block_params* p, const float* x, float* y,
                         const medt_block_saved* sv, void* ws, size_t ws_bytes, void* stream) {
    if (!d || !p || !x || !y || !sv) { set_error("block fwd: null argument"); return MEDT_EINVAL; }
    if (!wopos_block_ok(*d)) { set_error("block fwd: shape not supported by the fused kernel"); return MEDT_EUNSUPPORTED; }
    if (!p->w_down || !p->w_up || !p->height.w_qkv || !p->width.w_qkv || !sv->z1 || !sv->y1 || !sv->stats1 || !sv->y_h ||
        !sv->y_w || !sv->z2 || !sv->stats2 || !sv->height.qkv_raw || !sv->height.stacked || !sv->height.lse ||
        !sv->height.stats || !sv->width.qkv_raw || !sv->width.stacked || !sv->width.lse || !sv->width.stats) {
        set_error("block fwd: null pointer"); return MEDT_EINVAL;
    }
    const medt_bn_ptrs* bns[8] = {&p->bn1, &p->height.bn_qkv, &p->height.bn_similarity, &p->height.bn_output,
                                  &p->width.bn_qkv, &p->width.bn_similarity, &p->width.bn_output, &p->bn2};
    for (int b = 0; b < 8; ++b) {
        if (!bns[b]->weight || !bns[b]->bias) { set_error("block fwd: null BatchNorm parameter"); return MEDT_EINVAL; }
        if (!d->training && (!bns[b]->running_mean || !bns[b]->running_var)) {
            set_error("block fwd: eval mode needs running statistics"); return MEDT_EINVAL;
        }
    }
    Carver c(ws, ws_bytes);
    double* parts = c.take<double>(wopos_block_part_doubles(*d));
    if (!ws || !c.ok()) { set_error("block workspace too small: need %zu", c.off); return MEDT_EWORKSPACE; }
    hipStream_t s = (hipStream_t)stream;
    int rc = wopos_block_fwd(*d, *p, x, y, *sv, parts, s);
    if (rc) return rc;
    const int tr = d->training ? 1 : 0, gs = d->bn_groups, W = d->width, G = d->G;
    const double rows = (double)(d->N / gs) * d->H * d->W, sims = rows * d->H;
    AxialGeom gh;
    {
        medt_axial_desc ad{d->N, W, d->H, d->W, G, 0, 0, 1, d->training, gs, d->eps, d->momentum, 0, 0, 0};
        if ((rc = axial_geom(ad, &gh))) return rc;
    }
    LayerStats sh(sv->height.stats, gh), sw(sv->width.stats, gh);
    const int chs[8] = {W, 2 * W, G, W, 2 * W, G, W, d->C};
    const double cnt[8] = {rows, rows, sims, rows, rows, sims, rows, rows};
    BnStats outs[8] = {BnStats(sv->stats1, gs * W), sh.qkv, sh.sim, sh.out, sw.qkv, sw.sim, sw.out, BnStats(sv->stats2, gs * d->C)};
    const float* pp = reinterpret_cast<const float*>(parts);
    Queue* q = queue_for(s);
    for (int b = 0; b < 8; ++b) {
        if (q) q->fin.push_back(FinJob{make_fin(pp, 1, chs[b], cnt[b], *bns[b], outs[b]), gs, tr, d->momentum, d->eps});
        else if ((rc = bn_finalize(pp, 1, gs, chs[b], cnt[b], *bns[b], d->momentum, d->eps, tr, outs[b], s))) return rc;
        pp += (size_t)gs * chs[b] * 2 * 2;
    }
    return MEDT_OK;
}

size_t medt_wopos_block_s2_workspace_bytes(const medt_block_desc* d) {
    if (!d || !wopos_block_s2_ok(*d)) return 0;
    return align_up(wopos_block_s2_part_doubles(*d) * sizeof(double), 256) + 256;
}

int medt_wopos_block_s2_fwd(const medt_block_desc* d, const medt_block_s2_params* p, const float* x, float* y,
                            const medt_block_s2_saved* sv, void* ws, size_t ws_bytes, void* stream) {
    if (!d || !p || !x || !y || !sv) { set_error("block s2 fwd: null argument"); return MEDT_EINVAL; }
    if (!wopos_block_s2_ok(*d)) { set_error("block s2 fwd: shape not supported by the fused kernel"); return MEDT_EUNSUPPORTED; }
    const medt_block_params& bp = p->blk;
    const medt_block_saved& b0 = sv->blk;
    if (!bp.w_down || !bp.w_up || !bp.height.w_qkv || !bp.width.w_qkv || !p->w_ds || !b0.z1 || !b0.y1 || !b0.stats1 || !b0.y_h ||
        !b0.y_w || !b0.z2 || !b0.stats2 || !b0.height.qkv_raw || !b0.height.stacked || !b0.height.lse || !b0.height.stats ||
        !b0.width.qkv_raw || !b0.width.stacked || !b0.width.lse || !b0.width.stats || !sv->zd || !sv->yd || !sv->statsd) {
        set_error("block s2 fwd: null pointer"); return MEDT_EINVAL;
    }
    const medt_bn_ptrs* bns[9] = {&bp.bn1, &bp.height.bn_qkv, &bp.height.bn_similarity, &bp.height.bn_output,
                                  &bp.width.bn_qkv, &bp.width.bn_similarity, &bp.width.bn_output, &bp.bn2, &p->bn_ds};
    for (int b = 0; b < 9; ++b) {
        if (!bns[b]->weight || !bns[b]->bias) { set_error("block s2 fwd: null BatchNorm parameter"); return MEDT_EINVAL; }
        if (!d->training && (!bns[b]->running_mean || !bns[b]->running_var)) {
            set_error("block s2 fwd: eval mode needs running statistics"); return MEDT_EINVAL;
        }
    }
    Carver c(ws, ws_bytes);
    double* parts = c.take<double>(wopos_block_s2_part_doubles(*d));
    if (!ws || !c.ok()) { set_error("block s2 workspace too small: need %zu", c.off); return MEDT_EWORKSPACE; }
    hipStream_t s = (hipStream_t)stream;
    int rc = wopos_block_s2_fwd(*d, *p, x, y, *sv, parts, s);
    if (rc) return rc;
    const int tr = d->training ? 1 : 0, gs = d->bn_groups, W = d->width, G = d->G, CO = 2 * d->width;
    const double rows = (double)(d->N / gs) * d->H * d->W, sims = rows * d->H, rows2 = rows / 4;
    AxialGeom gh;
    {
        medt_axial_desc ad{d->N, W, d->H, d->W, G, 0, 0, 1, d->training, gs, d->eps, d->momentum, 0, 0, 0};
// ... 396 lines not shown
```

### medical-transformer_amd/csrc/medt_kernels.h

```cpp
#pragma once
#include "medt_common.h"

namespace medt {

struct Queue;

int conv1x1_ptiles(int HW);
int conv1x1_fwd(const float* x, const float* w, float* y, float* partials,
                int N, int Cin, int Cout, int HW, hipStream_t s);
int conv1x1_bwd_data(const float* dy, const float* raw, const float* coef, const float* w, float* dx,
                     int N, int Cin, int Cout, int HW, int groups, hipStream_t s);
struct TablesJob { const float* relative; float* tables; int HQ, L, blocks; };
int bn_finalize(const float* partials, int parts_per_group, int groups, int CH, double count,
                const medt_bn_ptrs& bn, float momentum, float eps, int training, BnStats out, hipStream_t s,
                const TablesJob* tables = nullptr);
int bn_finalize3(const float* p0, int CH0, double n0, const medt_bn_ptrs& bn0, BnStats o0,
                 const float* p1, int CH1, double n1, const medt_bn_ptrs& bn1, BnStats o1,
                 const float* p2, int CH2, double n2, const medt_bn_ptrs& bn2, BnStats o2,
                 int ppg, int groups, float momentum, float eps, int training, hipStream_t s);
int bn_bwd_finalize(const float* partials, int parts_per_group, int groups, int CH, double count, float dscale,
                    BnStats st, const float* weight, int training, float* coef, float* dweight, float* dbias,
                    hipStream_t s);

struct FinSrc;
// ... 26 lines not shown
int conv2d_bwd_data(const float* dy, const float* w, float* dx, float* wt_scratch, float* ksplit_scratch, int N, int Cin,
                    int H, int W, int Cout, int K, int stride, int pad, hipStream_t s, const float* add = nullptr, bool wt_ready = false);
bool conv2d_bwd_data_flips(int N, int Cin, int H, int W, int Cout, int K, int stride, int pad);
int conv_flip_weights(const float* w, float* wt, int Cout, int Cin, int K, hipStream_t s);
size_t conv2d_bwd_data_scratch_floats(int N, int Cin, int H, int W, int Cout, int K, int stride, int pad);
int conv2d_bwd_weight_splits(int N, int Cin, int Cout, int K, int Ho, int Wo);
int conv2d_bwd_weight(const float* dy, const float* raw, const float* coef, const float* x, float* dw, float* scratch,
                      int N, int Cin, int H, int W, int Cout, int K, int stride, int pad, int groups, hipStream_t s,
                      Queue* q = nullptr);
int channel_sum_splits_for(int N, int HW);
int channel_sum(const float* x, float* out, float* scratch , int N, int C, int HW, hipStream_t s);

bool conv_use_mfma(int Cin, int Cout, int K, int stride, long positions);
int conv_mfma_parts_per_group(int N, int groups, int HoWo);
bool conv_rows16_ok(int Cin, int H, int W, int K, int stride, int pad);
size_t conv_mfma_scratch_floats(int N, int groups, int HoWo, int Cin, int Cout, int K, bool rows16 = false);
int conv_mfma_fwd(const float* x, const float* w, const float* bias, float* y, float* partials, float* scratch, int N,
                  int Cin, int H, int W, int Cout, int K, int stride, int pad, int relu, int groups, hipStream_t s);
int conv_mfma_bwd_data_s1(const float* dy, const float* w, float* wt_scratch, float* ksplit_scratch, float* dx, int N,
                          int Cin, int H, int W, int Cout, int K, int pad, hipStream_t s, bool wt_ready = false);
int conv_wgrad_mfma(const float* dy, const float* raw, const float* coef, const float* x, float* scratch, int N, int Cin,
                    int H, int W, int Cout, int Ho, int Wo, int K, int stride, int pad, int QS, int splits, int npg,
                    hipStream_t s);

int bn_apply_act(const float* z, BnStats st, const float* res, float* y, int N, int C, int HW, int groups, int relu,
                 hipStream_t s);
int bn_act_bwd_stats(const float* dy, const float* y, const float* z, BnStats st, float* g, float* partials, int N, int C,
                     int HW, int groups, int relu, hipStream_t s);
int bn_bwd_apply(const float* g, const float* z, const float* coef, float* dz, int N, int C, int HW, int groups,
                 hipStream_t s);
int relu_mask(const float* a, const float* y, float* out, size_t total, hipStream_t s);
int seg_counts(const float* logits, const int64_t* target, int* counts, int N, int K, int HW, float threshold, hipStream_t s);
int relu_fwd(const float* x, float* y, size_t total, hipStream_t s);
int up2x_relu_add_fwd(const float* x, const float* skip, float* y, int NC, int H, int W, hipStream_t s);
int up2x_relu_bwd(const float* x, const float* dy, float* dx, int NC, int H, int W, hipStream_t s);
int patch_gather(const float* x, float* xp, int N, int C, int S, int P, int G, hipStream_t s);
int window_gather(const float* image, float* windows, const int32_t* oy, const int32_t* ox, int C, int H, int W, int S,
                  int ny, int nx, hipStream_t s);
int window_blend(const float* win, float* blended, uint8_t* mask, const int32_t* oy, const int32_t* ox, int K, int H, int W,
                 int S, int ny, int nx, float threshold, hipStream_t s);
size_t augment_param_floats();
int augment_parts(int th, int tw);
int augment_stats(const uint8_t* image, const float* params, float* workspace, int N, int H, int W, int C, int th, int tw,
                  hipStream_t s);
int augment_apply(const uint8_t* image, const uint8_t* mask, const float* params, float* workspace, float* out_image,
                  int64_t* out_mask, int N, int H, int W, int C, int th, int tw, int use_stats, hipStream_t s);
int edt_cols(const uint8_t* mask, int32_t* g2, int N, int H, int W, int border_mode, hipStream_t s);
int edt_rows(const int32_t* g2, const uint8_t* select, int32_t* d2, int N, int H, int W, hipStream_t s);
int signed_edt(const int64_t* target, int32_t* g2, int32_t* sd2, int N, int H, int W, int fg, int ignore, hipStream_t s);
size_t boundary_partials(int N, int HW);
size_t boundary_out_floats(int N);
int boundary_fwd(const float* logits, const int64_t* target, const int32_t* sd2, const float* alpha, const float* base,
                 float* partials, float* out, int N, int K, int HW, int fg, int ignore, hipStream_t s);
int boundary_bwd(const float* logits, const int64_t* target, const int32_t* sd2, const float* out, const float* dloss,
                 float* dlogits, int N, int K, int HW, int fg, int ignore, int accumulate, hipStream_t s);
int object_edt2(const int32_t* labels, int32_t* scratch, int32_t* d1sq, int32_t* d2sq, int N, int H, int W, hipStream_t s);
int border_fwd(const float* logits, const int64_t* target, const int32_t* d1sq, const int32_t* d2sq, float sigma, const float* w0,
               const float* base, float* partials, float* out, int N, int K, int HW, int fg, int ignore, hipStream_t s);
int border_bwd(const float* logits, const int64_t* target, const int32_t* d1sq, const int32_t* d2sq, float sigma, const float* out,
               const float* dloss, float* dlogits, int N, int K, int HW, int fg, int ignore, int accumulate, hipStream_t s);
size_t label_workspace_bytes(int N, int H, int W);
int label_components(const uint8_t* mask, int32_t* labels, int32_t* count, void* workspace, int N, int H, int W, int connectivity,
                     int background, hipStream_t s);
int label_tables(const int32_t* labels, int32_t* area, uint8_t* frame, int N, int H, int W, int stride, hipStream_t s);
int label_select(const int32_t* labels, const uint8_t* keep, const uint8_t* mask, uint8_t* out, int N, int H, int W, int stride,
                 hipStream_t s);
int label_boxes(const int32_t* labels, int32_t* box, int N, int H, int W, int stride, hipStream_t s);
int pair_hausdorff(const int32_t* la, const int32_t* lb, const int32_t* jobs, int32_t* scratch, int32_t* out, int n_jobs,
                   int col_blocks, int row_blocks, size_t scratch_elems, int n_out, int clear_out, int N, int H, int W, hipStream_t s);
int logo_merge_fwd(const float* x, const float* yp, float* y, int N, int C, int S, int P, int G, hipStream_t s);
int logo_merge_bwd(const float* dy, float* dx, float* dyp, int N, int C, int S, int P, int G, hipStream_t s);
int ce_parts(size_t npix);
int ce_fwd(const float* logits, const int64_t* target, float* partials, float* loss_out, int N, int K, int HW, int ignore,
           hipStream_t s);
int ce_bwd(const float* logits, const int64_t* target, const float* loss_out, const float* dloss, float* dlogits, int N,
           int K, int HW, int ignore, hipStream_t s);
int seg_loss_bpi(int HW);
size_t seg_loss_partials(int N, int K, int HW);
size_t seg_loss_out_floats(int N, int K);
int seg_loss_fwd(const float* logits, const int64_t* target, const float* weight, float* partials, float* out, int N, int K,
                 int HW, int ignore, float ce_scale, float dice_scale, float eps, hipStream_t s);
int seg_loss_bwd(const float* logits, const int64_t* target, const float* weight, const float* out, const float* dloss,
                 float* dlogits, int N, int K, int HW, int ignore, float ce_scale, float dice_scale, hipStream_t s);
int gate_sigmoid_fwd(const float* f_qr, const float* f_kr, const float* f_sve, const float* f_sv, float* eff, hipStream_t s);
int gate_sigmoid_bwd(const float* d_eff, const float* eff, float* dgate, hipStream_t s);
int gate_seq_reduce(const float* partials, float* dgates, int nseq, int G, hipStream_t s);
int gate_mlp_fwd(const float* x, const float* w1, const float* b1, const float* w2, const float* b2, float* xn, float* h,
                 float* o, float* gates, int N, int C, int H, int W, int axis, hipStream_t s);
int gate_mlp_bwd(const float* dgates, const float* gates, const float* o, const float* h, const float* xn, const float* w1,
                 const float* w2, float* d_o, float* dh, float* dxn, float* dw1, float* db1, float* dw2, float* db2,
                 float* dx, int N, int C, int H, int W, int axis, hipStream_t s);
int adam_step(float* p, const float* g, float* m, float* v, float* state, size_t n, float lr, float b1, float b2,
              float eps, float wd, float gscale, hipStream_t s);

struct AxialGeom {
    int N, C, H, W, G, gp, hq, L, Bo, axis, pos, OC, OCg, SC;
    int bf16;
    int groups, npg;
    int spg;
    int S_T;
    int tpg;
    int HW;
    int fast3;
    int fparts;
    int nt;
    int rows4, nt4, oparts;
    int bound_path;
    float bound_shift;
    double sim_count;
    double row_count;
};
int  axial_geom(const medt_axial_desc& d, AxialGeom* g);
size_t axial_core_lds_bytes(const AxialGeom& g, bool backward);

struct GatePtrs { const float *f_qr, *f_kr, *f_sve, *f_sv; int stride; };

struct FinSrc;
struct BfinSrc;
int axial_attn_fwd_fast(const AxialGeom& g, const float* qkv_raw, BnStats qkv, BnStats sim, const float* relative,
                        GatePtrs gates, float* stacked, float* lse, float* out_partials, unsigned* flag, hipStream_t s,
                        const FinSrc* simsrc = nullptr);
int axial_attn_fwd_fast_bf16(const AxialGeom& g, const float* qkv_raw, BnStats qkv, BnStats sim, const float* relative,
                             GatePtrs gates, float* stacked, float* lse, float* out_partials, unsigned* flag,
                             hipStream_t s, const FinSrc* simsrc = nullptr);
int fast3_max_subtiles(int gp, int L, int axis);
int fast4_subtile_sequences(int L);
int fast4_max_subtiles(int axis);
bool wopos_block_ok(const medt_block_desc& d);
size_t wopos_block_part_doubles(const medt_block_desc& d);
int wopos_block_fwd(const medt_block_desc& d, const medt_block_params& p, const float* x, float* y,
                    const medt_block_saved& sv, double* parts, hipStream_t s);
bool wopos_block_s2_ok(const medt_block_desc& d);
size_t wopos_block_s2_part_doubles(const medt_block_desc& d);
int wopos_block_s2_fwd(const medt_block_desc& d, const medt_block_s2_params& p, const float* x, float* y,
                       const medt_block_s2_saved& sv, double* parts, hipStream_t s);
bool wopos_block_bwd_ok(const medt_block_desc& d);
size_t wopos_block_bwd_ws_bytes(const medt_block_desc& d);
int wopos_block_bwd(const medt_block_desc& d, const medt_block_params& p, const float* x, const float* y, const float* dy,
                    const float* dx_add, const medt_block_saved& sv, float* dx, const medt_block_grads& gr, void* ws,
                    size_t ws_bytes, hipStream_t s);

bool conv_small_ok(const medt_conv_desc& d);
int conv_small_fwd(const medt_conv_desc& d, const float* x, const float* w, const medt_bn_ptrs& bn, const float* res,
                   float* z, float* y, float* partials, hipStream_t s);
bool bn_dgrad1x1_small_ok(const medt_conv_desc& d);
int bn_dgrad1x1_small(const medt_conv_desc& d, const float* dy, const float* y, const float* z, BnStats st,
                      const float* gamma, const float* w, const float* dx_add, float* g, float* dz, float* partials,
                      float* dx, hipStream_t s);
int bn_act_bwd_small(const medt_conv_desc& d, const float* dy, const float* y, const float* z, BnStats st,
                     const float* weight, float* g, float* dz, float* partials, int HoWo, hipStream_t s);
int bn_fin_apply(const float* z, const float* partials, int ppg, double count, const medt_bn_ptrs& bn, float eps, int training,
                 BnStats st, const float* res, float* y, int N, int C, int HW, int groups, int relu, hipStream_t s);
bool conv_fwd_ws_ok(int Cin, int Cout, int K, int stride, long positions);
int bn_chan_threads(const medt_conv_desc& d, int HoWo);
int bn_act_bwd_chan(const medt_conv_desc& d, const float* dy, const float* y, const float* z, BnStats st,
                    const float* weight, float* g, float* dz, float* partials, int HoWo, hipStream_t s);
bool wopos_small_ok(const AxialGeom& g, const medt_axial_desc& d);
int wopos_small_fwd(const AxialGeom& g, const medt_axial_desc& d, const medt_axial_params& p, const float* x, float* y,
                    float* qkv_raw, float* stacked, float* lse, float* part_q, float* part_s, float* part_o,
                    hipStream_t s);
bool wopos_small_bwd_ok(const AxialGeom& g, const medt_axial_desc& d);
int wopos_small_bwd(const AxialGeom& g, const medt_axial_desc& d, const medt_axial_params& p, const float* y,
                    const float* dy, const float* qkv_raw, const float* stacked, const float* lse, BnStats sq, BnStats ss,
                    BnStats so, float* dqkv, float* part_ob, float* part_sb, float* part_qb, float* coef_qkv,
                    hipStream_t s);
int wopos_small_bwd_finalize(const AxialGeom& g, const medt_axial_desc& d, const medt_axial_params& p,
                             const float* part_ob, const float* part_sb, const float* part_qb, BnStats sq, BnStats ss,
                             BnStats so, const medt_axial_grads& gr, hipStream_t s, Queue* q);
bool fast_path_enabled();

size_t sim_tables_floats(const AxialGeom& g);
int sim_tables_blocks(const AxialGeom& g);
int sim_stats_parts(const AxialGeom& g);
int axial_logit_stats(const AxialGeom& g, const float* qkv_raw, BnStats qkv, const float* relative, GatePtrs gates,
                      const float* tables, float* partials, hipStream_t s);
bool axial_attn_fwd_inlines(const AxialGeom& g, GatePtrs gates, const unsigned* flag);
int axial_attn_fwd(const AxialGeom& g, const float* qkv_raw, BnStats qkv, BnStats sim, const float* relative,
                   GatePtrs gates, float* stacked, float* lse, float* out_partials, unsigned* flag, hipStream_t s,
                   const FinSrc* simsrc = nullptr);
int axial_attn_bwd_stats(const AxialGeom& g, const float* qkv_raw, BnStats qkv, BnStats sim, const float* relative,
                         GatePtrs gates, const float* stacked, const float* lse, const float* dy,
                         const float* out_coef, int stride, float* partials, hipStream_t s);
int axial_sim_bwd_finalize(const AxialGeom& g, const float* partials, BnStats sim, const float* weight, int training,
                           float* coef, float* dweight, float* dbias, hipStream_t s, const TablesJob* tables = nullptr);
int axial_attn_bwd(const AxialGeom& g, const float* qkv_raw, BnStats qkv, BnStats sim, const float* sim_coef,
                   const float* relative, GatePtrs gates, const float* stacked, const float* lse, const float* dy,
                   const float* out_coef, int stride, float* dqkv, float* qkv_partials, float* rel_partials,
                   float* gate_partials, hipStream_t s);


struct SweepPlan {
    int LS, nw, S_T;
    int tiles, nparts;
    int fparts;
    int fix_ppt;
    int npg_floats;
    size_t lds;
};
bool axial_bwd_sweep_plan(const AxialGeom& g, int gate_stride, SweepPlan* p);
int axial_bwd_tables(const AxialGeom& g, const float* relative, float* tables, hipStream_t s);
int axial_attn_bwd_sweep(const AxialGeom& g, const SweepPlan& p, const float* qkv_raw, BnStats qkv, BnStats sim,
                         const float* relative, GatePtrs gates, const float* stacked, const float* lse, const float* dy,
                         const float* out_coef, int stride, float* dqkv, float* part_qb, int qb_rpg, float* part_sb,
                         float* rel_part, float* pg_part, float* gram, float* gate_raw, hipStream_t s, float* raw32 = nullptr,
                         const BfinSrc* ob = nullptr,
                         const float* ymask = nullptr);
int axial_attn_bwd_fix(const AxialGeom& g, const SweepPlan& p, const float* qkv_raw, BnStats qkv, const float* sim_coef,
                       const float* tables, const float* gram, GatePtrs gates, int apply, float* dqkv, float* part_qb,
                       int qb_rpg, hipStream_t s, const struct SimBSrc* sb = nullptr);
int axial_attn_bwd_relfix(const AxialGeom& g, const SweepPlan& p, const float* relative, const float* sim_coef, BnStats sim,
                          GatePtrs gates, const float* pg_part, const float* gate_raw, int training, float eps,
                          float* rel_rows, float* gate_rows, hipStream_t s, const BfinSrc* qb = nullptr);

}
```

### medical-transformer_amd/medt_amd/_lib.py

```python
from __future__ import annotations

import ctypes as C
import os

import torch

from .build import LIB_PATH

_lib = None
ABI_VERSION = 11


class MedtError(RuntimeError):
    pass


class AxialDesc(C.Structure):
    _fields_ = [("N", C.c_int32), ("C", C.c_int32), ("H", C.c_int32), ("W", C.c_int32), ("G", C.c_int32),
                ("axis", C.c_int32), ("has_pos", C.c_int32), ("stride", C.c_int32), ("training", C.c_int32),
                ("bn_groups", C.c_int32), ("eps", C.c_float), ("momentum", C.c_float), ("out_relu", C.c_int32),
                ("gate_mode", C.c_int32), ("act_dtype", C.c_int32)]


class ConvDesc(C.Structure):
    _fields_ = [("N", C.c_int32), ("Cin", C.c_int32), ("H", C.c_int32), ("W", C.c_int32), ("Cout", C.c_int32),
                ("K", C.c_int32), ("stride", C.c_int32), ("pad", C.c_int32), ("has_bias", C.c_int32),
                ("has_bn", C.c_int32), ("has_res", C.c_int32), ("relu", C.c_int32), ("training", C.c_int32),
                ("bn_groups", C.c_int32), ("eps", C.c_float), ("momentum", C.c_float), ("lean", C.c_int32)]


class BnPtrs(C.Structure):
    _fields_ = [("weight", C.c_void_p), ("bias", C.c_void_p), ("running_mean", C.c_void_p),
                ("running_var", C.c_void_p), ("num_batches_tracked", C.c_void_p)]


class AxialParams(C.Structure):
    _fields_ = [("w_qkv", C.c_void_p), ("bn_qkv", BnPtrs), ("bn_similarity", BnPtrs), ("bn_output", BnPtrs),
                ("relative", C.c_void_p), ("f_qr", C.c_void_p), ("f_kr", C.c_void_p), ("f_sve", C.c_void_p),
                ("f_sv", C.c_void_p)]


class AxialSaved(C.Structure):
    _fields_ = [("qkv_raw", C.c_void_p), ("stacked", C.c_void_p), ("lse", C.c_void_p), ("stats", C.c_void_p)]


class AxialGrads(C.Structure):
    _fields_ = [("w_qkv", C.c_void_p), ("bn_qkv_weight", C.c_void_p), ("bn_qkv_bias", C.c_void_p),
                ("bn_sim_weight", C.c_void_p), ("bn_sim_bias", C.c_void_p), ("bn_out_weight", C.c_void_p),
                ("bn_out_bias", C.c_void_p), ("relative", C.c_void_p), ("gates", C.c_void_p)]


class BlockDesc(C.Structure):
    _fields_ = [("N", C.c_int32), ("C", C.c_int32), ("width", C.c_int32), ("H", C.c_int32), ("W", C.c_int32),
                ("G", C.c_int32), ("training", C.c_int32), ("bn_groups", C.c_int32), ("eps", C.c_float),
                ("momentum", C.c_float)]


class BlockParams(C.Structure):
    _fields_ = [("w_down", C.c_void_p), ("bn1", BnPtrs), ("height", AxialParams), ("width", AxialParams),
                ("w_up", C.c_void_p), ("bn2", BnPtrs)]


class BlockSaved(C.Structure):
    _fields_ = [("z1", C.c_void_p), ("y1", C.c_void_p), ("stats1", C.c_void_p), ("height", AxialSaved),
                ("y_h", C.c_void_p), ("width", AxialSaved), ("y_w", C.c_void_p), ("z2", C.c_void_p),
                ("stats2", C.c_void_p)]


class BlockS2Params(C.Structure):
    _fields_ = [("blk", BlockParams), ("w_ds", C.c_void_p), ("bn_ds", BnPtrs)]


class BlockS2Saved(C.Structure):
    _fields_ = [("blk", BlockSaved), ("zd", C.c_void_p), ("yd", C.c_void_p), ("statsd", C.c_void_p)]


class BlockGrads(C.Structure):
    _fields_ = [("w_down", C.c_void_p), ("bn1_weight", C.c_void_p), ("bn1_bias", C.c_void_p), ("height", AxialGrads),
                ("width", AxialGrads), ("w_up", C.c_void_p), ("bn2_weight", C.c_void_p), ("bn2_bias", C.c_void_p)]


SIGNATURES = {
    "medt_abi_version": (C.c_int, []),
    "medt_last_error": (C.c_char_p, []),
    "medt_queue_create": (C.c_void_p, []),
    "medt_queue_destroy": (C.c_int, [C.c_void_p]),
    "medt_queue_bind": (C.c_int, [C.c_void_p, C.c_void_p]),
    "medt_queue_pending": (C.c_size_t, [C.c_void_p]),
    "medt_queue_flush": (C.c_int, [C.c_void_p, C.c_void_p]),
    "medt_queue_flush2": (C.c_int, [C.c_void_p, C.c_void_p, C.c_void_p]),
    "medt_queue_discard": (C.c_int, [C.c_void_p]),
    "medt_axial_stats_floats": (C.c_size_t, [C.POINTER(AxialDesc)]),
    "medt_axial_workspace_bytes": (C.c_size_t, [C.POINTER(AxialDesc)]),
    "medt_axial_layer_fwd": (C.c_int, [C.POINTER(AxialDesc), C.POINTER(AxialParams), C.c_void_p, C.c_void_p,
                                       C.POINTER(AxialSaved), C.c_void_p, C.c_size_t, C.c_void_p]),
    "medt_axial_layer_bwd": (C.c_int, [C.POINTER(AxialDesc), C.POINTER(AxialParams), C.c_void_p, C.c_void_p, C.c_void_p,
                                       C.POINTER(AxialSaved), C.c_void_p, C.POINTER(AxialGrads), C.c_void_p,
                                       C.c_size_t, C.c_void_p]),
    "medt_axial_core_stats": (C.c_int, [C.POINTER(AxialDesc), C.POINTER(AxialParams), C.POINTER(AxialSaved),
                                        C.c_void_p, C.c_size_t, C.c_void_p]),
    "medt_axial_core_fwd": (C.c_int, [C.POINTER(AxialDesc), C.POINTER(AxialParams), C.POINTER(AxialSaved),
                                      C.c_void_p, C.c_size_t, C.c_void_p]),
    "medt_axial_core_bwd": (C.c_int, [C.POINTER(AxialDesc), C.POINTER(AxialParams), C.POINTER(AxialSaved), C.c_void_p,
                                      C.c_void_p, C.c_size_t, C.c_void_p]),
    "medt_wopos_block_workspace_bytes": (C.c_size_t, [C.POINTER(BlockDesc)]),
    "medt_wopos_block_fwd": (C.c_int, [C.POINTER(BlockDesc), C.POINTER(BlockParams), C.c_void_p, C.c_void_p,
                                       C.POINTER(BlockSaved), C.c_void_p, C.c_size_t, C.c_void_p]),
    "medt_wopos_block_s2_workspace_bytes": (C.c_size_t, [C.POINTER(BlockDesc)]),
    "medt_wopos_block_s2_fwd": (C.c_int, [C.POINTER(BlockDesc), C.POINTER(BlockS2Params), C.c_void_p, C.c_void_p,
                                          C.POINTER(BlockS2Saved), C.c_void_p, C.c_size_t, C.c_void_p]),
    "medt_wopos_block_bwd_workspace_bytes": (C.c_size_t, [C.POINTER(BlockDesc)]),
    "medt_wopos_block_bwd": (C.c_int, [C.POINTER(BlockDesc), C.POINTER(BlockParams), C.c_void_p, C.c_void_p, C.c_void_p,
                                       C.POINTER(BlockSaved), C.c_void_p, C.c_void_p, C.POINTER(BlockGrads), C.c_void_p,
                                       C.c_size_t, C.c_void_p]),
    "medt_conv_stats_floats": (C.c_size_t, [C.POINTER(ConvDesc)]),
    "medt_conv_workspace_bytes": (C.c_size_t, [C.POINTER(ConvDesc)]),
    "medt_conv_block_fwd": (C.c_int, [C.POINTER(ConvDesc), C.c_void_p, C.c_void_p, C.c_void_p, C.POINTER(BnPtrs),
                                      C.c_void_p, C.c_void_p, C.c_void_p, C.c_void_p, C.c_void_p, C.c_size_t, C.c_void_p]),
    "medt_conv_block_bwd": (C.c_int, [C.POINTER(ConvDesc), C.c_void_p, C.c_void_p, C.POINTER(BnPtrs), C.c_void_p,
                                      C.c_void_p, C.c_void_p, C.c_void_p, C.c_void_p, C.c_void_p, C.c_void_p, C.c_void_p,
                                      C.c_void_p, C.c_void_p, C.c_void_p, C.c_void_p, C.c_size_t, C.c_void_p]),
    "medt_gate_mlp_fwd": (C.c_int, [C.c_void_p] * 9 + [C.c_int] * 5 + [C.c_void_p]),
    "medt_gate_mlp_bwd": (C.c_int, [C.c_void_p] * 13 + [C.c_int] * 5 + [C.c_void_p]),
    "medt_up2x_relu_add_fwd": (C.c_int, [C.c_void_p, C.c_void_p, C.c_void_p, C.c_int, C.c_int, C.c_int, C.c_void_p]),
    "medt_up2x_relu_bwd": (C.c_int, [C.c_void_p, C.c_void_p, C.c_void_p, C.c_int, C.c_int, C.c_int, C.c_void_p]),
    "medt_patch_gather": (C.c_int, [C.c_void_p, C.c_void_p, C.c_int, C.c_int, C.c_int, C.c_int, C.c_int, C.c_void_p]),
    "medt_logo_merge_fwd": (C.c_int, [C.c_void_p, C.c_void_p, C.c_void_p, C.c_int, C.c_int, C.c_int, C.c_int, C.c_int,
                                      C.c_void_p]),
    "medt_logo_merge_bwd": (C.c_int, [C.c_void_p, C.c_void_p, C.c_void_p, C.c_int, C.c_int, C.c_int, C.c_int, C.c_int,
                                      C.c_void_p]),
    "medt_ce_partials": (C.c_size_t, [C.c_int, C.c_int]),
    "medt_ce_fwd": (C.c_int, [C.c_void_p, C.c_void_p, C.c_void_p, C.c_void_p, C.c_int, C.c_int, C.c_int, C.c_int,
                              C.c_void_p]),
    "medt_ce_bwd": (C.c_int, [C.c_void_p, C.c_void_p, C.c_void_p, C.c_void_p, C.c_void_p, C.c_int, C.c_int, C.c_int,
                              C.c_int, C.c_void_p]),
    "medt_seg_loss_workspace": (C.c_size_t, [C.c_int, C.c_int, C.c_int]),
    "medt_seg_loss_out_floats": (C.c_size_t, [C.c_int, C.c_int]),
    "medt_seg_loss_fwd": (C.c_int, [C.c_void_p] * 5 + [C.c_int] * 4 + [C.c_float] * 3 + [C.c_void_p]),
    "medt_seg_loss_bwd": (C.c_int, [C.c_void_p] * 6 + [C.c_int] * 4 + [C.c_float] * 3 + [C.c_void_p]),
    "medt_adam_step": (C.c_int, [C.c_void_p, C.c_void_p, C.c_void_p, C.c_void_p, C.c_void_p, C.c_size_t, C.c_float,
                                 C.c_float, C.c_float, C.c_float, C.c_float, C.c_float, C.c_void_p]),
    "medt_relu_mask": (C.c_int, [C.c_void_p, C.c_void_p, C.c_void_p, C.c_size_t, C.c_void_p]),
    "medt_seg_counts": (C.c_int, [C.c_void_p, C.c_void_p, C.c_void_p, C.c_int, C.c_int, C.c_int, C.c_float, C.c_void_p]),
    "medt_window_gather": (C.c_int, [C.c_void_p] * 4 + [C.c_int] * 6 + [C.c_void_p]),
    "medt_window_blend": (C.c_int, [C.c_void_p] * 5 + [C.c_int] * 6 + [C.c_float, C.c_void_p]),
    "medt_augment_param_floats": (C.c_size_t, []),
    "medt_augment_workspace": (C.c_size_t, [C.c_int, C.c_int, C.c_int]),
    "medt_augment_stats": (C.c_int, [C.c_void_p] * 3 + [C.c_int] * 6 + [C.c_void_p]),
    "medt_augment_apply": (C.c_int, [C.c_void_p] * 6 + [C.c_int] * 7 + [C.c_void_p]),
    "medt_edt_cols": (C.c_int, [C.c_void_p] * 2 + [C.c_int] * 4 + [C.c_void_p]),
    "medt_edt_rows": (C.c_int, [C.c_void_p] * 3 + [C.c_int] * 3 + [C.c_void_p]),
    "medt_signed_edt": (C.c_int, [C.c_void_p] * 3 + [C.c_int] * 5 + [C.c_void_p]),
    "medt_boundary_workspace": (C.c_size_t, [C.c_int, C.c_int]),
    "medt_boundary_out_floats": (C.c_size_t, [C.c_int]),
    "medt_boundary_fwd": (C.c_int, [C.c_void_p] * 7 + [C.c_int] * 5 + [C.c_void_p]),
    "medt_boundary_bwd": (C.c_int, [C.c_void_p] * 6 + [C.c_int] * 6 + [C.c_void_p]),
    "medt_object_edt2": (C.c_int, [C.c_void_p] * 4 + [C.c_int] * 3 + [C.c_void_p]),
    "medt_border_workspace": (C.c_size_t, [C.c_int, C.c_int]),
    "medt_border_out_floats": (C.c_size_t, [C.c_int]),
    "medt_border_fwd": (C.c_int, [C.c_void_p] * 4 + [C.c_float] + [C.c_void_p] * 4 + [C.c_int] * 5 + [C.c_void_p]),
    "medt_border_bwd": (C.c_int, [C.c_void_p] * 4 + [C.c_float] + [C.c_void_p] * 3 + [C.c_int] * 6 + [C.c_void_p]),
    "medt_label_workspace_bytes": (C.c_size_t, [C.c_int] * 3),
    "medt_label_components": (C.c_int, [C.c_void_p] * 4 + [C.c_size_t] + [C.c_int] * 5 + [C.c_void_p]),
    "medt_label_tables": (C.c_int, [C.c_void_p] * 3 + [C.c_int] * 5 + [C.c_void_p]),
    "medt_label_select": (C.c_int, [C.c_void_p] * 4 + [C.c_int] * 4 + [C.c_void_p]),
    "medt_label_boxes": (C.c_int, [C.c_void_p] * 2 + [C.c_int] * 5 + [C.c_void_p]),
    "medt_pair_hausdorff": (C.c_int, [C.c_void_p] * 5 + [C.c_int] * 3 + [C.c_size_t] + [C.c_int] * 5 + [C.c_void_p]),
}


def lib():
    global _lib
    if _lib is None:
        if not os.path.exists(LIB_PATH):
            raise MedtError(f"{LIB_PATH} not found: build it with `python __graft_entry__.py` "
                            "(hipcc --offload-arch=gfx950); there is no CPU / eager fallback")
        l = C.CDLL(os.environ.get("MEDT_LIB_OVERRIDE", LIB_PATH))
        for name, (res, args) in SIGNATURES.items():
            fn = getattr(l, name)
            fn.restype = res
            fn.argtypes = args
        if l.medt_abi_version() != ABI_VERSION:
            raise MedtError("libmedt_hip.so ABI version mismatch")
        _lib = l
    return _lib


def check(rc: int, what: str):
    if rc != 0:
        raise MedtError(f"{what} failed ({rc}): {lib().medt_last_error().decode()}")


def ptr(t):
    return None if t is None else t.data_ptr()
```

### medical-transformer_amd/medt_amd/net.py

```python
from __future__ import annotations

import torch

from ._lib import MedtError
from . import ops
from . import defer as DEFER
from . import block as BLOCK

import os

PATCH = 32
GRID = 4
TWO_STREAMS = os.environ.get("MEDT_TWO_STREAMS", "1") != "0"
SINKS = os.environ.get("MEDT_GRAD_SINKS", "1") != "0"
EARLY_FIN = os.environ.get("MEDT_EARLY_FIN", "1") != "0"
_side = {}


def _side_stream(device):
    key = (device.type, device.index)
    if key not in _side:
        _side[key] = torch.cuda.Stream(device=device)
    return _side[key]


def join_side_stream(device):
    side = _side.get((device.type, device.index))
    if side is not None:
        torch.cuda.current_stream().wait_stream(side)


def _require_device(x):
    if not x.is_cuda:
        raise MedtError("medt_amd runs on MI355X only: got a CPU tensor and there is no CPU fallback "
                        "(the CPU restatement under oracle/ is test infrastructure)")


def axial_block_forward(blk, x, bn_groups: int = 1):
    _require_device(x)
    sink = ops.sink_of(x) if (SINKS and x.requires_grad) else None
    if BLOCK.BWD_ENABLED:
        y = BLOCK.block_forward(blk, x, bn_groups, sink)
        if y is not None:
            return y
    pre = BLOCK.fused_forward(blk, x, bn_groups)
    if pre is None:
        pre = {"down": None, "h": None, "w": None, "up": None}
    pre.setdefault("ds", None)
    out = ops.conv_block(x, blk.conv_down, blk.bn1, relu=True, training=blk.bn1.training, bn_groups=bn_groups,
                         x_sink=sink, x_role="final", pre=pre["down"])
    out = blk.hight_block.run(out, bn_groups, False, pre["h"])
    out = blk.width_block.run(out, bn_groups, True, pre["w"])
    if blk.downsample is not None:
        identity = ops.conv_block(x, blk.downsample[0], blk.downsample[1], relu=False,
                                  training=blk.downsample[1].training, bn_groups=bn_groups, x_sink=sink, x_role="deposit",
                                  pre=pre["ds"])
        return ops.conv_block(out, blk.conv_up, blk.bn2, res=identity, relu=True, training=blk.bn2.training,
                              bn_groups=bn_groups, pre=pre["up"])
    return ops.conv_block(out, blk.conv_up, blk.bn2, res=x, relu=True, training=blk.bn2.training,
                          bn_groups=bn_groups, res_sink=sink, pre=pre["up"])


def _layer(seq, x, bn_groups=1):
    for blk in seq:
        x = axial_block_forward(blk, x, bn_groups)
    return x


def _stem(net, x, sfx="", bn_groups=1, first_of_branch=False):
    g = lambda n: getattr(net, n + sfx)
    for i in ("1", "2", "3"):
        bn = g("bn" + i)
        x = ops.conv_block(x, g("conv" + i), bn, relu=True, training=bn.training, bn_groups=bn_groups,
                           last_of_branch=first_of_branch and i == "1")
    return x


def _unet_body(net, x, sfx="", bn_groups=1):
    g = lambda n: getattr(net, n + sfx)
    x1 = _layer(g("layer1"), x, bn_groups)
    x2 = _layer(g("layer2"), x1, bn_groups)
    x3 = _layer(g("layer3"), x2, bn_groups)
    x4 = _layer(g("layer4"), x3, bn_groups)
    sk = (lambda t: ops.sink_of(t)) if SINKS else (lambda t: None)
    y = ops.up2x_relu_add(ops.conv_block(x4, g("decoder1")), x4)
    y = ops.up2x_relu_add(ops.conv_block(y, g("decoder2")), x3, sk(x3))
    y = ops.up2x_relu_add(ops.conv_block(y, g("decoder3")), x2, sk(x2))
    y = ops.up2x_relu_add(ops.conv_block(y, g("decoder4")), x1, sk(x1))
    y = ops.up2x_relu_add(ops.conv_block(y, g("decoder5")), None)
    return y


def unet_forward(net, x):
    _require_device(x)
    y = _unet_body(net, _stem(net, x.contiguous()))
    return ops.conv_block(y, net.adjust)


def medt_forward(net, x):
    _require_device(x)
    xin = x.contiguous()
    if xin.shape[2] < PATCH * GRID or xin.shape[3] < PATCH * GRID or xin.shape[2] != xin.shape[3]:
        raise RuntimeError(f"medt_net needs square images of at least {PATCH * GRID} px (4x4 grid of 32-px patches)")
    main = torch.cuda.current_stream()
    side = _side_stream(xin.device) if TWO_STREAMS else None
    if side is not None:
        side.wait_stream(main)
    DEFER.set_aux_stream(side)
    g = _stem(net, xin, first_of_branch=side is not None)
    x1 = _layer(net.layer1, g)
    x2 = _layer(net.layer2, x1)
    y = ops.up2x_relu_add(ops.conv_block(x2, net.decoder4), x1, ops.sink_of(x1) if SINKS else None)
    y = ops.up2x_relu_add(ops.conv_block(y, net.decoder5), None)
    if side is not None and EARLY_FIN:
        DEFER.flush_current_stream()
    groups = GRID * GRID
    ops.set_lean(side is not None and xin.shape[2] * xin.shape[3] > 128 * 128)
    try:
        if side is not None:
            with torch.cuda.stream(side):
                xp = ops.patch_gather(xin, PATCH, GRID)
                yp = _unet_body(net, _stem(net, xp, "_p", groups), "_p", groups)
                if EARLY_FIN:
                    joined = torch.cuda.Event()
                    joined.record(side)
                    DEFER.flush_current_stream()
            if EARLY_FIN:
                main.wait_event(joined)
            else:
                main.wait_stream(side)
            yp.record_stream(main)
        else:
            xp = ops.patch_gather(xin, PATCH, GRID)
            yp = _unet_body(net, _stem(net, xp, "_p", groups), "_p", groups)
    finally:
        ops.set_lean(False)
    y = ops.logo_merge(y, yp, PATCH, GRID)
    y = ops.conv_block(y, net.decoderf, relu=True)
    return ops.conv_block(y, net.adjust)
```

### medical-transformer_amd/medt_amd/ops.py

```python
from __future__ import annotations

import ctypes as C
import os

import torch

from . import _lib as L
from . import optim as OPT
from . import defer as DEFER
from .axial import _bn_ptrs, _momentum, _require_device


def _stream():
    return torch.cuda.current_stream().cuda_stream


class GradSink:
    __slots__ = ("pending", "closed")

    def __init__(self):
        self.pending, self.closed = None, False

    def deposit(self, t) -> bool:
        if self.closed or self.pending is not None:
            return False
        self.pending = t
        return True

    def take(self):
        t, self.pending = self.pending, None
        return t


def sink_of(x):
    s = getattr(x, "_medt_sink", None)
    if s is None:
        s = x._medt_sink = GradSink()
    return s


import threading
_hint = threading.local()


def set_lean(v: bool):
    _hint.lean = bool(v)


def lean() -> bool:
    return getattr(_hint, "lean", False)



class ConvBlockCfg:
    __slots__ = ("stride", "pad", "bn", "relu", "bn_groups", "x_sink", "x_role", "res_sink", "last_of_branch", "pre", "lean")

    def __init__(self, stride, pad, bn, relu, bn_groups=1, x_sink=None, x_role=None, res_sink=None, last_of_branch=False,
                 pre=None):
        self.stride, self.pad, self.bn, self.relu, self.bn_groups = stride, pad, bn, relu, bn_groups
        self.x_sink, self.x_role, self.res_sink = x_sink, x_role, res_sink
        self.last_of_branch = last_of_branch
        self.pre = pre
        self.lean = lean()


def _conv_desc(x, w, cfg: ConvBlockCfg, has_bias, has_res, training) -> L.ConvDesc:
    N, Cin, H, W = x.shape
    bn = cfg.bn
    return L.ConvDesc(N, Cin, H, W, w.shape[0], w.shape[2], cfg.stride, cfg.pad, int(has_bias), int(bn is not None),
                      int(has_res), int(cfg.relu), int(training), cfg.bn_groups,
                      bn.eps if bn is not None else 1e-5,
                      _momentum(bn) if bn is not None else 0.1, int(cfg.lean))


class ConvBlockFn(torch.autograd.Function):
    @staticmethod
    def forward(ctx, x, w, bias, bn_w, bn_b, res, cfg: ConvBlockCfg, training: bool):
        _require_device(x)
        lib = L.lib()
        x = x.contiguous()
        if res is not None:
            res = res.contiguous()
        desc = _conv_desc(x, w, cfg, bias is not None, res is not None, training)
        K, s, p = w.shape[2], cfg.stride, cfg.pad
        N, _, H, W = x.shape
        Ho, Wo = (H + 2 * p - K) // s + 1, (W + 2 * p - K) // s + 1
        has_bn = cfg.bn is not None
        if cfg.pre is not None:
            z, y, stats = cfg.pre
            cfg.pre = None
        else:
            y = torch.empty((N, w.shape[0], Ho, Wo), device=x.device, dtype=torch.float32)
            z = torch.empty_like(y) if has_bn else y
            stats = torch.empty((max(lib.medt_conv_stats_floats(C.byref(desc)), 1),), device=x.device, dtype=torch.float32)
            ws_bytes = lib.medt_conv_workspace_bytes(C.byref(desc))
            if ws_bytes == 0:
                raise L.MedtError("conv block: " + lib.medt_last_error().decode())
            ws = torch.empty((ws_bytes,), device=x.device, dtype=torch.uint8)
            bnp = _bn_ptrs(cfg.bn, training) if has_bn else None
            q = DEFER.recording() if (has_bn or stats.numel() > 1) else None
            L.check(lib.medt_conv_block_fwd(C.byref(desc), x.data_ptr(), w.data_ptr(), L.ptr(bias),
                                            C.byref(bnp) if has_bn else None, L.ptr(res), z.data_ptr(), y.data_ptr(),
                                            stats.data_ptr(), ws.data_ptr(), ws_bytes, _stream()), "medt_conv_block_fwd")
            if q is not None:
                q.hold(ws, stats)
        ctx.cfg, ctx.training, ctx.has_bias, ctx.has_res = cfg, training, bias is not None, res is not None
        ctx.slots = tuple(OPT.grad_slot(t) if t is not None else None for t in (w, bias, bn_w, bn_b))
        ctx.save_for_backward(x, w, z if has_bn else None, y if (cfg.relu or has_bn) else None,
                              stats if (has_bn or stats.numel() > 1) else None)
        return y

    @staticmethod
    def backward(ctx, dy):
        lib = L.lib()
        x, w, z, y, stats = ctx.saved_tensors
        cfg, training = ctx.cfg, ctx.training
        dy = dy.contiguous()
        desc = _conv_desc(x, w, cfg, ctx.has_bias, ctx.has_res, training)
        has_bn = cfg.bn is not None
        dev = x.device
        Cout = w.shape[0]
        need_dx = ctx.needs_input_grad[0]
        dx = torch.empty_like(x) if need_dx else None
        xs = cfg.x_sink if need_dx else None
        dep = xs.take() if xs is not None else None
        dx_add = dep if (dep is not None and w.shape[2] == 1) else None
        present = (True, ctx.has_bias, has_bn, has_bn)
        shapes = (w.shape, (Cout,), (Cout,), (Cout,))
        dst, ret, pend = [None] * 4, [None] * 4, []
        for k in range(4):
            if not present[k]:
                continue
            slot = OPT.live(ctx.slots[k])
            if slot is not None and ctx.needs_input_grad[k + 1]:
                dst[k], direct = OPT.claim(slot)
                if not direct:
                    pend.append((slot, dst[k]))
            else:
                dst[k] = torch.empty(shapes[k], device=dev, dtype=torch.float32)
                if ctx.needs_input_grad[k + 1]:
                    ret[k] = dst[k]
        dres = torch.empty_like(dy) if ctx.has_res else None
        ws_bytes = lib.medt_conv_workspace_bytes(C.byref(desc))
        ws = torch.empty((ws_bytes,), device=dev, dtype=torch.uint8)
        bnp = _bn_ptrs(cfg.bn, False) if has_bn else None
        q = DEFER.recording(allow=not pend and all(r is None for r in ret))
        L.check(lib.medt_conv_block_bwd(C.byref(desc), x.data_ptr(), w.data_ptr(), C.byref(bnp) if has_bn else None,
                                        L.ptr(z), L.ptr(y), L.ptr(stats), dy.data_ptr(), L.ptr(dx), dst[0].data_ptr(),
                                        L.ptr(dst[1]), L.ptr(dst[2]), L.ptr(dst[3]), L.ptr(dres), L.ptr(dx_add), ws.data_ptr(),
                                        ws_bytes, _stream()), "medt_conv_block_bwd")
        if q is not None:
            q.hold(ws, x, dy, stats, dres, *dst)
        for slot, tmp in pend:
            OPT.accumulate(slot, tmp)
        if dep is not None and dx_add is None:
            dx.add_(dep)
        if xs is not None:
            if cfg.x_role == "final":
                xs.closed = True
            elif xs.deposit(dx):
                dx = None
        if dres is not None and cfg.res_sink is not None and cfg.res_sink.deposit(dres):
            dres = None
        if cfg.last_of_branch:
            if DEFER.flush_current_stream():
                OPT.branch_done(0)
        return (dx, ret[0], ret[1], ret[2], ret[3], dres, None, None)


def conv_block(x, conv, bn=None, res=None, relu=False, training=False, bn_groups=1, x_sink=None, x_role=None,
               res_sink=None, last_of_branch=False, pre=None):
    cfg = ConvBlockCfg(conv.stride[0], conv.padding[0], bn, relu, bn_groups if bn is not None else 1, x_sink, x_role,
                       res_sink, last_of_branch, pre)
    if bn is None:
        training = torch.is_grad_enabled() and (x.requires_grad or conv.weight.requires_grad)
    return ConvBlockFn.apply(x, conv.weight, conv.bias, bn.weight if bn is not None else None,
                             bn.bias if bn is not None else None, res, cfg, training)


class UpReluAddFn(torch.autograd.Function):
    @staticmethod
    def forward(ctx, x, skip, skip_sink=None):
        ctx.skip_sink = skip_sink
        _require_device(x)
        lib = L.lib()
        x = x.contiguous()
        N, Cc, H, W = x.shape
        y = torch.empty((N, Cc, 2 * H, 2 * W), device=x.device, dtype=torch.float32)
        if skip is not None:
            skip = skip.contiguous()
        L.check(lib.medt_up2x_relu_add_fwd(x.data_ptr(), L.ptr(skip), y.data_ptr(), N * Cc, H, W, _stream()),
                "medt_up2x_relu_add_fwd")
        ctx.save_for_backward(x)
        ctx.has_skip = skip is not None
        return y

    @staticmethod
    def backward(ctx, dy):
        lib = L.lib()
        (x,) = ctx.saved_tensors
        dy = dy.contiguous()
        N, Cc, H, W = x.shape
        dx = torch.empty_like(x)
        L.check(lib.medt_up2x_relu_bwd(x.data_ptr(), dy.data_ptr(), dx.data_ptr(), N * Cc, H, W, _stream()),
                "medt_up2x_relu_bwd")
        dskip = dy if ctx.has_skip else None
        if dskip is not None and ctx.skip_sink is not None and ctx.skip_sink.deposit(dskip):
            dskip = None
        return dx, dskip, None


def up2x_relu_add(x, skip=None, skip_sink=None):
    return UpReluAddFn.apply(x, skip, skip_sink)


class GateMlpFn(torch.autograd.Function):

    @staticmethod
    def forward(ctx, x, w1, b1, w2, b2, axis):
        _require_device(x)
        lib = L.lib()
        x = x.contiguous()
        N, Cc, H, W = x.shape
        nseq = N * (H if axis else W)
        dev = x.device
        xn = torch.empty((nseq, Cc), device=dev, dtype=torch.float32)
        h = torch.empty_like(xn)
        o = torch.empty((nseq, 4), device=dev, dtype=torch.float32)
        gates = torch.empty_like(o)
        L.check(lib.medt_gate_mlp_fwd(x.data_ptr(), w1.data_ptr(), b1.data_ptr(), w2.data_ptr(), b2.data_ptr(),
                                      xn.data_ptr(), h.data_ptr(), o.data_ptr(), gates.data_ptr(), N, Cc, H, W, axis,
                                      _stream()), "medt_gate_mlp_fwd")
        ctx.save_for_backward(w1, w2, xn, h, o, gates)
        ctx.geom = (N, Cc, H, W, axis)
        return gates

    @staticmethod
    def backward(ctx, dgates):
        lib = L.lib()
        w1, w2, xn, h, o, gates = ctx.saved_tensors
        N, Cc, H, W, axis = ctx.geom
        dev = dgates.device
        nseq = gates.shape[0]
        dgates = dgates.contiguous()
        scratch = torch.empty((nseq * (4 + 2 * Cc),), device=dev, dtype=torch.float32)
        dw1, db1 = torch.empty_like(w1), torch.empty((Cc,), device=dev, dtype=torch.float32)
        dw2, db2 = torch.empty_like(w2), torch.empty((4,), device=dev, dtype=torch.float32)
        dx = torch.empty((N, Cc, H, W), device=dev, dtype=torch.float32)
        L.check(lib.medt_gate_mlp_bwd(dgates.data_ptr(), gates.data_ptr(), o.data_ptr(), h.data_ptr(), xn.data_ptr(),
                                      w1.data_ptr(), w2.data_ptr(), scratch.data_ptr(), dw1.data_ptr(), db1.data_ptr(),
                                      dw2.data_ptr(), db2.data_ptr(), dx.data_ptr(), N, Cc, H, W, axis, _stream()),
                "medt_gate_mlp_bwd")
        return dx, dw1, db1, dw2, db2, None


def gate_mlp(x, fcn1, fcn2, width: bool):
    return GateMlpFn.apply(x, fcn1.weight, fcn1.bias, fcn2.weight, fcn2.bias, 1 if width else 0)


def patch_gather(x, P=32, G=4):
    _require_device(x)
    x = x.contiguous()
    N, Cc, S, _ = x.shape
    xp = torch.empty((G * G * N, Cc, P, P), device=x.device, dtype=torch.float32)
    L.check(L.lib().medt_patch_gather(x.data_ptr(), xp.data_ptr(), N, Cc, S, P, G, _stream()), "medt_patch_gather")
    return xp


class LogoMergeFn(torch.autograd.Function):
    @staticmethod
    def forward(ctx, x, yp, P, G):
        _require_device(x)
        x, yp = x.contiguous(), yp.contiguous()
        N, Cc, S, _ = x.shape
        y = torch.empty_like(x)
        L.check(L.lib().medt_logo_merge_fwd(x.data_ptr(), yp.data_ptr(), y.data_ptr(), N, Cc, S, P, G, _stream()),
                "medt_logo_merge_fwd")
        ctx.geom = (N, Cc, S, P, G)
        return y

    @staticmethod
    def backward(ctx, dy):
        N, Cc, S, P, G = ctx.geom
        dy = dy.contiguous()
        dx = torch.empty_like(dy)
        dyp = torch.empty((G * G * N, Cc, P, P), device=dy.device, dtype=torch.float32)
        L.check(L.lib().medt_logo_merge_bwd(dy.data_ptr(), dx.data_ptr(), dyp.data_ptr(), N, Cc, S, P, G, _stream()),
                "medt_logo_merge_bwd")
        return dx, dyp, None, None


def logo_merge(x, yp, P=32, G=4):
    return LogoMergeFn.apply(x, yp, P, G)


class CrossEntropyFn(torch.autograd.Function):
    @staticmethod
    def forward(ctx, logits, target, ignore_index):
        _require_device(logits)
        lib = L.lib()
        logits, target = logits.contiguous(), target.contiguous()
        if target.dtype != torch.int64:
            raise L.MedtError("cross_entropy: int64 class-index targets expected")
        N, K = logits.shape[0], logits.shape[1]
        HW = logits[0, 0].numel()
        partials = torch.empty((lib.medt_ce_partials(N, HW),), device=logits.device, dtype=torch.float32)
        out = torch.empty((3,), device=logits.device, dtype=torch.float32)
        L.check(lib.medt_ce_fwd(logits.data_ptr(), target.data_ptr(), partials.data_ptr(), out.data_ptr(), N, K, HW,
                                ignore_index, _stream()), "medt_ce_fwd")
        ctx.save_for_backward(logits, target, out)
        ctx.ignore_index = ignore_index
        loss = out[0]
        ctx.mark_non_differentiable(out)
        ctx.set_materialize_grads(False)
        return loss, out

    @staticmethod
    def backward(ctx, dloss, _dout):
        if dloss is None:
            return None, None, None
        lib = L.lib()
        logits, target, out = ctx.saved_tensors
        N, K = logits.shape[0], logits.shape[1]
        HW = logits[0, 0].numel()
        dloss = dloss.contiguous().float()
        dlogits = torch.empty_like(logits)
        L.check(lib.medt_ce_bwd(logits.data_ptr(), target.data_ptr(), out.data_ptr(), dloss.data_ptr(),
                                dlogits.data_ptr(), N, K, HW, ctx.ignore_index, _stream()), "medt_ce_bwd")
        return dlogits, None, None

# ... 651 lines not shown
```

Measured before the change: 2162 images/s.

## Batch conv_down and downsample 1x1 conv+BN forwards into paired launches

Adds a paired forward path that runs the two 1x1 conv+BN blocks reading the same input (conv_down and downsample) through a single launch each for the conv, the small-conv fused kernel and the BN finalize/apply. Kernel bodies are factored into device functions and dispatched by block index onto one of two jobs. The aim is to cut kernel launch count and fill the GPU better for these small batch-4 problems. The cost is extra host-side workspace allocation in Python and more code paths to maintain.

```diff
diff --git a/include/medt_abi.h b/include/medt_abi.h
--- a/include/medt_abi.h
+++ b/include/medt_abi.h
@@ -168,6 +168,12 @@
 int medt_conv_block_fwd(const medt_conv_desc*, const float* x, const float* w, const float* bias,
                         const medt_bn_ptrs* bn, const float* res, float* z, float* y, float* stats,
                         void* workspace, size_t workspace_bytes, void* stream);
+int medt_conv_block_pair_fwd(const medt_conv_desc* da, const float* xa, const float* wa, const float* biasa,
+                             const medt_bn_ptrs* bna, const float* resa, float* za, float* ya, float* statsa,
+                             void* workspace_a, size_t workspace_a_bytes,
+                             const medt_conv_desc* db, const float* xb, const float* wb, const float* biasb,
+                             const medt_bn_ptrs* bnb, const float* resb, float* zb, float* yb, float* statsb,
+                             void* workspace_b, size_t workspace_b_bytes, void* stream);
 int medt_conv_block_bwd(const medt_conv_desc*, const float* x, const float* w, const medt_bn_ptrs* bn,
                         const float* z, const float* y, const float* stats, const float* dy,
                         float* dx, float* dw, float* dbias, float* dbn_weight, float* dbn_bias, float* dres,
diff --git a/medical-transformer_amd/csrc/conv.hip b/medical-transformer_amd/csrc/conv.hip
--- a/medical-transformer_amd/csrc/conv.hip
+++ b/medical-transformer_amd/csrc/conv.hip
@@ -4,14 +4,13 @@
 namespace medt {
 
 template <int K, int OT>
-__global__ __launch_bounds__(MEDT_THREADS) void conv2d_fwd_kernel(
+__device__ __forceinline__ void conv2d_fwd_body(
     const float* __restrict__ x, const float* __restrict__ w, const float* __restrict__ bias, float* __restrict__ y,
     float* __restrict__ partials, int Cin, int H, int W, int Cout, int Ho, int Wo, int stride, int pad, int relu,
-    int npg, int y_bf16) {
+    int npg, int y_bf16, float* red, int bx, int by) {
     constexpr int KK = K * K;
-    MEDT_STATIC_SHARED float red[MEDT_WAVES * OT * 2 * 2];
     const int HoWo = Ho * Wo, per_group = npg * HoWo, ppg = (per_group + MEDT_THREADS - 1) / MEDT_THREADS;
-    const int grp = blockIdx.x / ppg, part = blockIdx.x - grp * ppg, o0 = blockIdx.y * OT;
+    const int grp = bx / ppg, part = bx - grp * ppg, o0 = by * OT;
     const int q = part * MEDT_THREADS + threadIdx.x;
     const bool ok = q < per_group;
     const int ni = ok ? q / HoWo : 0, p = ok ? q - ni * HoWo : 0;
@@ -70,8 +69,36 @@
             v[2 * o] = a;
             v[2 * o + 1] = a * a;
         }
-        block_sum_d<2 * OT>(v, red, reinterpret_cast<double*>(partials) + ((size_t)blockIdx.x * Cout + o0) * 2);
-    }
+        block_sum_d<2 * OT>(v, red, reinterpret_cast<double*>(partials) + ((size_t)bx * Cout + o0) * 2);
+    }
+}
+
+template <int K, int OT>
+__global__ __launch_bounds__(MEDT_THREADS) void conv2d_fwd_kernel(
+    const float* __restrict__ x, const float* __restrict__ w, const float* __restrict__ bias, float* __restrict__ y,
+    float* __restrict__ partials, int Cin, int H, int W, int Cout, int Ho, int Wo, int stride, int pad, int relu,
+    int npg, int y_bf16) {
+    MEDT_STATIC_SHARED float red[MEDT_WAVES * OT * 2 * 2];
+    conv2d_fwd_body<K, OT>(x, w, bias, y, partials, Cin, H, W, Cout, Ho, Wo, stride, pad, relu, npg, y_bf16, red, blockIdx.x,
+                           blockIdx.y);
+}
+
+struct ConvFwdJob {
+    const float *x, *w;
+    float *y, *partials;
+    int Cin, H, W, Cout, Ho, Wo, stride, pad, npg, gx;
+};
+struct ConvFwdPair { ConvFwdJob job[2]; int blocksA; };
+
+template <int OT>
+__global__ __launch_bounds__(MEDT_THREADS) void conv1x1_fwd_pair_kernel(ConvFwdPair p) {
+    MEDT_STATIC_SHARED float red[MEDT_WAVES * OT * 2 * 2];
+    const int second = (int)blockIdx.x >= p.blocksA ? 1 : 0;
+    const ConvFwdJob& j = p.job[second];
+    const int local = (int)blockIdx.x - (second ? p.blocksA : 0);
+    const int by = local / j.gx, bx = local - by * j.gx;
+    conv2d_fwd_body<1, OT>(j.x, j.w, nullptr, j.y, j.partials, j.Cin, j.H, j.W, j.Cout, j.Ho, j.Wo, j.stride, j.pad, 0, j.npg, 0,
+                           red, bx, by);
 }
 
 int conv2d_parts_per_group(int N, int groups, int HoWo) { return cdiv((N / groups) * HoWo, MEDT_THREADS); }
@@ -272,6 +299,46 @@
     }
     set_error("conv2d: kernel size %d unsupported (1, 3, 7)", K);
     return MEDT_EUNSUPPORTED;
+}
+
+bool conv1x1_fwd_plain(int N, int groups, int Cin, int H, int W, int Cout, int K, int stride, int pad) {
+    if (K != 1 || pad != 0 || stride < 1) return false;
+    const int Ho = (H - 1) / stride + 1, Wo = (W - 1) / stride + 1;
+    const long pos = (long)N * Ho * Wo;
+    if (conv_stem7_ok(Cin, H, W, Cout, K, stride, pad) || conv_use_mfma(Cin, Cout, K, stride, pos)) return false;
+    if ((conv_thin_mode() & 1) && conv_thin_ok(N, groups, Cin, H, W, Cout, K, stride, pad)) return false;
+    return !conv_fwd_ws_ok(Cin, Cout, K, stride, pos);
+}
+
+int conv1x1_fwd_pair(const Conv1x1Problem& a, const Conv1x1Problem& b, hipStream_t s) {
+    if (abl_skip(a.N >= 16 ? "conv1_fwd_l" : "conv1_fwd_g")) return MEDT_OK;
+    const Conv1x1Problem* in[2] = {&a, &b};
+    ConvFwdPair p;
+    int tile = 16;
+    for (int i = 0; i < 2; ++i) {
+        const Conv1x1Problem& q = *in[i];
+        ConvFwdJob& j = p.job[i];
+        j.x = q.x; j.w = q.w; j.y = q.y; j.partials = q.partials;
+        j.Cin = q.Cin; j.H = q.H; j.W = q.W; j.Cout = q.Cout; j.stride = q.stride; j.pad = 0;
+        j.Ho = (q.H - 1) / q.stride + 1; j.Wo = (q.W - 1) / q.stride + 1;
+        j.npg = q.N / q.groups;
+        j.gx = q.groups * conv2d_parts_per_group(q.N, q.groups, j.Ho * j.Wo);
+        const int t = pick_tile(q.Cout, 16, j.gx);
+        if (t < tile) tile = t;
+    }
+    while (a.Cout % tile || b.Cout % tile) tile >>= 1;
+    p.blocksA = p.job[0].gx * (a.Cout / tile);
+    const unsigned blocks = (unsigned)(p.blocksA + p.job[1].gx * (b.Cout / tile));
+#define MEDT_LAUNCH_PAIR(OT) hipLaunchKernelGGL(conv1x1_fwd_pair_kernel<OT>, dim3(blocks), dim3(MEDT_THREADS), 0, s, p)
+    switch (tile) {
+        case 16: MEDT_LAUNCH_PAIR(16); break;
+        case 8: MEDT_LAUNCH_PAIR(8); break;
+        case 4: MEDT_LAUNCH_PAIR(4); break;
+        case 2: MEDT_LAUNCH_PAIR(2); break;
+        default: MEDT_LAUNCH_PAIR(1); break;
+    }
+#undef MEDT_LAUNCH_PAIR
+    return launch_status("conv1x1_fwd_pair");
 }
 
 template <int K, int CT>
diff --git a/medical-transformer_amd/csrc/conv_small.hip b/medical-transformer_amd/csrc/conv_small.hip
--- a/medical-transformer_amd/csrc/conv_small.hip
+++ b/medical-transformer_amd/csrc/conv_small.hip
@@ -60,9 +60,8 @@
 }
 
 template <int T, int SC_NOC>
-__global__ __launch_bounds__(T) void conv1x1_bn_small_fwd_kernel(SmallConvArgs a) {
-    extern __shared__ __attribute__((aligned(16))) float smem[];
-    const int grp = blockIdx.x, oc0 = blockIdx.y * SC_NOC, tid = threadIdx.x, lane = tid & 63, wave = tid >> 6;
+__device__ __forceinline__ void conv1x1_bn_small_fwd_body(const SmallConvArgs& a, float* smem, int bx, int by) {
+    const int grp = bx, oc0 = by * SC_NOC, tid = threadIdx.x, lane = tid & 63, wave = tid >> 6;
     constexpr int NW = T >> 6;
     const int Cin = a.Cin, W = a.W, HW = a.H * a.W, st = a.stride, Ho = a.H / st, Wo = a.W / st, HoWo = Ho * Wo;
     const int P = a.npg * HoWo, n0 = grp * a.npg;
@@ -227,6 +226,22 @@
     }
 }
 
+template <int T, int SC_NOC>
+__global__ __launch_bounds__(T) void conv1x1_bn_small_fwd_kernel(SmallConvArgs a) {
+    extern __shared__ __attribute__((aligned(16))) float smem[];
+    conv1x1_bn_small_fwd_body<T, SC_NOC>(a, smem, blockIdx.x, blockIdx.y);
+}
+
+struct SmallConvPair { SmallConvArgs job[2]; int gx[2]; int blocksA; };
+template <int T, int SC_NOC>
+__global__ __launch_bounds__(T) void conv1x1_bn_small_fwd_pair_kernel(SmallConvPair p) {
+    extern __shared__ __attribute__((aligned(16))) float smem[];
+    const int second = (int)blockIdx.x >= p.blocksA ? 1 : 0;
+    const int local = (int)blockIdx.x - (second ? p.blocksA : 0), gx = p.gx[second];
+    const int by = local / gx;
+    conv1x1_bn_small_fwd_body<T, SC_NOC>(p.job[second], smem, local - by * gx, by);
+}
+
 static size_t conv_small_lds(int P, int Cin, int noc) {
     const int ks = conv_small_ksplit(P, Cin);
     return ((size_t)noc * P + (size_t)Cin * noc + 8 * noc + (ks > 1 ? (size_t)ks * noc * P : 0)) * sizeof(float);
@@ -256,14 +271,52 @@
     return true;
 }
 
-int conv_small_fwd(const medt_conv_desc& d, const float* x, const float* w, const medt_bn_ptrs& bn, const float* res,
-                   float* z, float* y, float* partials, hipStream_t s) {
-    if (abl_skip("conv_small_fwd")) return MEDT_OK;
+static SmallConvArgs conv_small_args(const medt_conv_desc& d, const float* x, const float* w, const medt_bn_ptrs& bn, const float* res,
+                                     float* z, float* y, float* partials) {
     SmallConvArgs a;
     a.x = x; a.w = w; a.res = d.has_res ? res : nullptr; a.bn = bn; a.z = z; a.y = y; a.partials = partials;
     a.N = d.N; a.Cin = d.Cin; a.H = d.H; a.W = d.W; a.Cout = d.Cout; a.stride = d.stride; a.npg = d.N / d.bn_groups;
     a.relu = d.relu; a.training = d.training ? 1 : 0; a.eps = d.eps;
-    const int P = a.npg * (d.H / d.stride) * (d.W / d.stride);
+    return a;
+}
+static int conv_small_positions(const medt_conv_desc& d) { return (d.N / d.bn_groups) * (d.H / d.stride) * (d.W / d.stride); }
+
+bool conv_small_pair_ok(const medt_conv_desc& a, const medt_conv_desc& b) {
+    const int Pa = conv_small_positions(a), Pb = conv_small_positions(b);
+    return conv_small_threads(Pa) == conv_small_threads(Pb) && conv_small_noc(Pa, a.Cin) == conv_small_noc(Pb, b.Cin);
+}
+
+int conv_small_fwd_pair(const medt_conv_desc& da, const float* xa, const float* wa, const medt_bn_ptrs& bna, const float* resa,
+                        float* za, float* ya, float* partialsa, const medt_conv_desc& db, const float* xb, const float* wb,
+                        const medt_bn_ptrs& bnb, const float* resb, float* zb, float* yb, float* partialsb, hipStream_t s) {
+    if (abl_skip("conv_small_fwd")) return MEDT_OK;
+    SmallConvPair p;
+    p.job[0] = conv_small_args(da, xa, wa, bna, resa, za, ya, partialsa);
+    p.job[1] = conv_small_args(db, xb, wb, bnb, resb, zb, yb, partialsb);
+    const int Pa = conv_small_positions(da), Pb = conv_small_positions(db);
+    const int threads = conv_small_threads(Pa), noc = conv_small_noc(Pa, da.Cin);
+    p.gx[0] = da.bn_groups;
+    p.gx[1] = db.bn_groups;
+    p.blocksA = da.bn_groups * (da.Cout / noc);
+    const dim3 grid((unsigned)(p.blocksA + db.bn_groups * (db.Cout / noc)));
+    const size_t la = conv_small_lds(Pa, da.Cin, noc), lb = conv_small_lds(Pb, db.Cin, noc), lds = la > lb ? la : lb;
+#define MEDT_SMALL_PAIR(TT)                                                                                   \
+    do {                                                                                                      \
+        if (noc == 16) hipLaunchKernelGGL((conv1x1_bn_small_fwd_pair_kernel<TT, 16>), grid, dim3(TT), lds, s, p); \
+        else hipLaunchKernelGGL((conv1x1_bn_small_fwd_pair_kernel<TT, 8>), grid, dim3(TT), lds, s, p);         \
+    } while (0)
+    if (threads == 256) MEDT_SMALL_PAIR(256);
+    else if (threads == 512) MEDT_SMALL_PAIR(512);
+    else MEDT_SMALL_PAIR(1024);
+#undef MEDT_SMALL_PAIR
+    return launch_status("conv1x1_bn_small_fwd_pair");
+}
+
+int conv_small_fwd(const medt_conv_desc& d, const float* x, const float* w, const medt_bn_ptrs& bn, const float* res,
+                   float* z, float* y, float* partials, hipStream_t s) {
+    if (abl_skip("conv_small_fwd")) return MEDT_OK;
+    const SmallConvArgs a = conv_small_args(d, x, w, bn, res, z, y, partials);
+    const int P = conv_small_positions(d);
     const int threads = conv_small_threads(P);
     const int noc = conv_small_noc(P, d.Cin);
     const dim3 grid(d.bn_groups, d.Cout / noc);
diff --git a/medical-transformer_amd/csrc/elementwise.hip b/medical-transformer_amd/csrc/elementwise.hip
--- a/medical-transformer_amd/csrc/elementwise.hip
+++ b/medical-transformer_amd/csrc/elementwise.hip
@@ -38,9 +38,8 @@
     float eps;
 };
 constexpr int BFA_PER_THREAD = 16;
-__global__ __launch_bounds__(MEDT_THREADS) void bn_fin_apply_kernel(BnFinApplyArgs a) {
-    MEDT_STATIC_SHARED double redd[2 * MEDT_WAVES];
-    const int grp = blockIdx.x / a.parts, part = blockIdx.x - grp * a.parts, c = blockIdx.y, tid = threadIdx.x;
+__device__ __forceinline__ void bn_fin_apply_body(const BnFinApplyArgs& a, double* redd, int bx, int by) {
+    const int grp = bx / a.parts, part = bx - grp * a.parts, c = by, tid = threadIdx.x;
     const int gc = grp * a.C + c;
     const float gam = a.weight[c], bet = a.bias[c];
     float mean_f, rstd_f, scale, shift;
@@ -112,16 +111,51 @@
     }
 }
 
-int bn_fin_apply(const float* z, const float* partials, int ppg, double count, const medt_bn_ptrs& bn, float eps, int training,
-                 BnStats st, const float* res, float* y, int N, int C, int HW, int groups, int relu, hipStream_t s) {
+__global__ __launch_bounds__(MEDT_THREADS) void bn_fin_apply_kernel(BnFinApplyArgs a) {
+    MEDT_STATIC_SHARED double redd[2 * MEDT_WAVES];
+    bn_fin_apply_body(a, redd, blockIdx.x, blockIdx.y);
+}
+
+struct BnFinApplyPair { BnFinApplyArgs job[2]; int gx[2]; int blocksA; };
+__global__ __launch_bounds__(MEDT_THREADS) void bn_fin_apply_pair_kernel(BnFinApplyPair p) {
+    MEDT_STATIC_SHARED double redd[2 * MEDT_WAVES];
+    const int second = (int)blockIdx.x >= p.blocksA ? 1 : 0;
+    const int local = (int)blockIdx.x - (second ? p.blocksA : 0), gx = p.gx[second];
+    const int by = local / gx;
+    bn_fin_apply_body(p.job[second], redd, local - by * gx, by);
+}
+
+static BnFinApplyArgs bn_fin_apply_args(const float* z, const float* partials, int ppg, double count, const medt_bn_ptrs& bn, float eps,
+                                        int training, BnStats st, const float* res, float* y, int N, int C, int HW, int groups,
+                                        int relu) {
     BnFinApplyArgs a;
     a.z = z; a.partials = partials; a.weight = bn.weight; a.bias = bn.bias; a.running_mean = bn.running_mean;
     a.running_var = bn.running_var; a.res = res; a.y = y; a.st = st; a.C = C; a.HW = HW; a.npg = N / groups; a.ppg = ppg;
     a.parts = cdiv(a.npg * HW, MEDT_THREADS * BFA_PER_THREAD); a.relu = relu; a.training = training; a.count = count;
     a.vec4 = ((HW & 3) == 0 && (((uintptr_t)z | (uintptr_t)y | (uintptr_t)res) & 15) == 0) ? 1 : 0;
     a.eps = eps;
+    return a;
+}
+
+int bn_fin_apply(const float* z, const float* partials, int ppg, double count, const medt_bn_ptrs& bn, float eps, int training,
+                 BnStats st, const float* res, float* y, int N, int C, int HW, int groups, int relu, hipStream_t s) {
+    const BnFinApplyArgs a = bn_fin_apply_args(z, partials, ppg, count, bn, eps, training, st, res, y, N, C, HW, groups, relu);
     hipLaunchKernelGGL(bn_fin_apply_kernel, dim3(groups * a.parts, C), dim3(MEDT_THREADS), 0, s, a);
     return launch_status("bn_fin_apply");
+}
+
+int bn_fin_apply_pair(const BnFinApplyProblem& a, const BnFinApplyProblem& b, hipStream_t s) {
+    const BnFinApplyProblem* in[2] = {&a, &b};
+    BnFinApplyPair p;
+    for (int i = 0; i < 2; ++i) {
+        const BnFinApplyProblem& q = *in[i];
+        p.job[i] = bn_fin_apply_args(q.z, q.partials, q.ppg, q.count, *q.bn, q.eps, q.training, q.st, q.res, q.y, q.N, q.C, q.HW,
+                                     q.groups, q.relu);
+        p.gx[i] = q.groups * p.job[i].parts;
+    }
+    p.blocksA = p.gx[0] * a.C;
+    hipLaunchKernelGGL(bn_fin_apply_pair_kernel, dim3((unsigned)(p.blocksA + p.gx[1] * b.C)), dim3(MEDT_THREADS), 0, s, p);
+    return launch_status("bn_fin_apply_pair");
 }
 
 __global__ __launch_bounds__(MEDT_THREADS) void bn_act_bwd_stats_kernel(const float* __restrict__ dy,
diff --git a/medical-transformer_amd/csrc/medt_api.hip b/medical-transformer_amd/csrc/medt_api.hip
--- a/medical-transformer_amd/csrc/medt_api.hip
+++ b/medical-transformer_amd/csrc/medt_api.hip
@@ -512,59 +512,141 @@
     return align_up(c.off, 256) + 256;
 }
 
+}
+
+namespace medt {
+struct ConvFwdCall {
+    const medt_conv_desc* d;
+    const float *x, *w, *bias;
+    const medt_bn_ptrs* bn;
+    const float* res;
+    float *z, *y, *stats;
+    void* ws;
+    size_t ws_bytes;
+    ConvGeom g;
+    float *partials, *ksplit_fwd;
+    int tr;
+    double count;
+
+    int check() {
+        int rc = conv_geom(d, &g);
+        if (rc) return rc;
+        if (!x || !w || !y || (d->has_bias && !bias) || (d->has_bn && (!bn || !z || !stats)) || (d->has_res && !res)) {
+            set_error("conv fwd: null pointer"); return MEDT_EINVAL;
+        }
+        Carver c(ws, ws_bytes);
+        ConvWs cw(c, d, g);
+        if (!ws || !c.ok()) { set_error("conv workspace too small: need %zu", c.off); return MEDT_EWORKSPACE; }
+        partials = cw.partials;
+        ksplit_fwd = cw.ksplit_fwd;
+        tr = d->training ? 1 : 0;
+        count = d->has_bn ? (double)(d->N / d->bn_groups) * g.HoWo : 0.0;
+        return MEDT_OK;
+    }
+    int check_bn() const {
+        if (!tr && (!bn->running_mean || !bn->running_var)) { set_error("conv fwd: eval mode needs running statistics"); return MEDT_EINVAL; }
+        if (tr && count <= 1.0) {
+            set_error("conv fwd: training-mode BatchNorm needs more than 1 value per channel"); return MEDT_EINVAL;
+        }
+        return MEDT_OK;
+    }
+    BnStats st() const { return BnStats(stats, d->bn_groups * d->Cout); }
+    int preflip(hipStream_t s) const;
+    int finish_small(hipStream_t s) const {
+        if (Queue* q = queue_for(s)) {
+            q->fin.push_back(FinJob{make_fin(partials, 1, d->Cout, count, *bn, st()), d->bn_groups, tr, d->momentum, d->eps});
+            return MEDT_OK;
+        }
+        return bn_finalize(partials, 1, d->bn_groups, d->Cout, count, *bn, d->momentum, d->eps, tr, st(), s);
+    }
+    int finish_generic(hipStream_t s) const {
+        if (!tr) return MEDT_OK;
+        if (Queue* q = queue_for(s)) {
+            q->fin.push_back(FinJob{make_fin(partials, g.ppg, d->Cout, count, *bn, st()), d->bn_groups, 2, d->momentum, d->eps});
+            return MEDT_OK;
+        }
+        return bn_finalize(partials, g.ppg, d->bn_groups, d->Cout, count, *bn, d->momentum, d->eps, 2, st(), s);
+    }
+    BnFinApplyProblem apply_problem() const {
+        return BnFinApplyProblem{z, partials, d->has_res ? res : nullptr, bn, y, st(), g.ppg, d->N, d->Cout, g.HoWo, d->bn_groups,
+                                 d->relu, tr, count, d->eps};
+    }
+    int run(hipStream_t s) const;
+};
+}
+
+extern "C" {
+
+int medt::ConvFwdCall::preflip(hipStream_t s) const {
+    if (!(stats && conv_preflip(d))) return MEDT_OK;
+    float* wt = conv_preflip_ptr(d, stats);
+    if (Queue* q = queue_for(s)) { q->flip.push_back(FlipJob{w, wt, d->Cout, d->Cin, d->K}); return MEDT_OK; }
+    return conv_flip_weights(w, wt, d->Cout, d->Cin, d->K, s);
+}
+
+int medt::ConvFwdCall::run(hipStream_t s) const {
+    int rc = preflip(s);
+    if (rc) return rc;
+    if (!d->has_bn)
+        return conv2d_fwd(x, w, d->has_bias ? bias : nullptr, y, nullptr, ksplit_fwd, d->N, d->Cin, d->H, d->W, d->Cout,
+                          d->K, d->stride, d->pad, d->relu, 1, s);
+    if ((rc = check_bn())) return rc;
+    if (conv_small_ok(*d)) {
+        if ((rc = conv_small_fwd(*d, x, w, *bn, res, z, y, partials, s))) return rc;
+        return finish_small(s);
+    }
+    if ((rc = conv2d_fwd(x, w, nullptr, z, tr ? partials : nullptr, ksplit_fwd, d->N, d->Cin, d->H, d->W, d->Cout, d->K,
+                         d->stride, d->pad, 0, d->bn_groups, s))) return rc;
+    static const bool fused_fin = true;
+    if (!fused_fin) {
+        if ((rc = bn_finalize(partials, g.ppg, d->bn_groups, d->Cout, count, *bn, d->momentum, d->eps, tr, st(), s))) return rc;
+        return bn_apply_act(z, st(), d->has_res ? res : nullptr, y, d->N, d->Cout, g.HoWo, d->bn_groups, d->relu, s);
+    }
+    if ((rc = bn_fin_apply(z, partials, g.ppg, count, *bn, d->eps, tr, st(), d->has_res ? res : nullptr, y, d->N, d->Cout,
+                           g.HoWo, d->bn_groups, d->relu, s))) return rc;
+    return finish_generic(s);
+}
+
 int medt_conv_block_fwd(const medt_conv_desc* d, const float* x, const float* w, const float* bias,
                         const medt_bn_ptrs* bn, const float* res, float* z, float* y, float* stats, void* ws,
                         size_t ws_bytes, void* stream) {
-    ConvGeom g;
-    int rc = conv_geom(d, &g);
+    ConvFwdCall c{d, x, w, bias, bn, res, z, y, stats, ws, ws_bytes};
+    int rc = c.check();
     if (rc) return rc;
-    if (!x || !w || !y || (d->has_bias && !bias) || (d->has_bn && (!bn || !z || !stats)) || (d->has_res && !res)) {
-        set_error("conv fwd: null pointer"); return MEDT_EINVAL;
-    }
+    return c.run((hipStream_t)stream);
+}
+
+int medt_conv_block_pair_fwd(const medt_conv_desc* da, const float* xa, const float* wa, const float* biasa,
+                             const medt_bn_ptrs* bna, const float* resa, float* za, float* ya, float* statsa, void* wsa,
+                             size_t wsa_bytes, const medt_conv_desc* db, const float* xb, const float* wb, const float* biasb,
+                             const medt_bn_ptrs* bnb, const float* resb, float* zb, float* yb, float* statsb, void* wsb,
+                             size_t wsb_bytes, void* stream) {
+    ConvFwdCall a{da, xa, wa, biasa, bna, resa, za, ya, statsa, wsa, wsa_bytes};
+    ConvFwdCall b{db, xb, wb, biasb, bnb, resb, zb, yb, statsb, wsb, wsb_bytes};
+    int rc;
+    if ((rc = a.check()) || (rc = b.check())) return rc;
     hipStream_t s = (hipStream_t)stream;
-    Carver c(ws, ws_bytes);
-    ConvWs cw(c, d, g);
-    if (!ws || !c.ok()) { set_error("conv workspace too small: need %zu", c.off); return MEDT_EWORKSPACE; }
-    if (stats && conv_preflip(d)) {
-        float* wt = conv_preflip_ptr(d, stats);
-        if (Queue* q = queue_for(s)) q->flip.push_back(FlipJob{w, wt, d->Cout, d->Cin, d->K});
-        else if ((rc = conv_flip_weights(w, wt, d->Cout, d->Cin, d->K, s))) return rc;
-    }
-    if (!d->has_bn)
-        return conv2d_fwd(x, w, d->has_bias ? bias : nullptr, y, nullptr, cw.ksplit_fwd, d->N, d->Cin, d->H, d->W, d->Cout,
-                          d->K, d->stride, d->pad, d->relu, 1, s);
-    const int tr = d->training ? 1 : 0;
-    if (!tr && (!bn->running_mean || !bn->running_var)) { set_error("conv fwd: eval mode needs running statistics"); return MEDT_EINVAL; }
-    if (tr && (double)(d->N / d->bn_groups) * g.HoWo <= 1.0) {
-        set_error("conv fwd: training-mode BatchNorm needs more than 1 value per channel"); return MEDT_EINVAL;
-    }
-    BnStats st(stats, d->bn_groups * d->Cout);
-    if (conv_small_ok(*d)) {
-        if ((rc = conv_small_fwd(*d, x, w, *bn, res, z, y, cw.partials, s))) return rc;
-        if (Queue* q = queue_for(s)) {
-            q->fin.push_back(FinJob{make_fin(cw.partials, 1, d->Cout, (double)(d->N / d->bn_groups) * g.HoWo, *bn, st),
-                                    d->bn_groups, tr, d->momentum, d->eps});
-            return MEDT_OK;
-        }
-        return bn_finalize(cw.partials, 1, d->bn_groups, d->Cout, (double)(d->N / d->bn_groups) * g.HoWo, *bn, d->momentum,
-                           d->eps, tr, st, s);
-    }
-    if ((rc = conv2d_fwd(x, w, nullptr, z, tr ? cw.partials : nullptr, cw.ksplit_fwd, d->N, d->Cin, d->H, d->W, d->Cout, d->K,
-                         d->stride, d->pad, 0, d->bn_groups, s))) return rc;
-    static const bool fused_fin = true;
-    const double count = (double)(d->N / d->bn_groups) * g.HoWo;
-    if (!fused_fin) {
-        if ((rc = bn_finalize(cw.partials, g.ppg, d->bn_groups, d->Cout, count, *bn, d->momentum, d->eps, tr, st, s))) return rc;
-        return bn_apply_act(z, st, d->has_res ? res : nullptr, y, d->N, d->Cout, g.HoWo, d->bn_groups, d->relu, s);
-    }
-    if ((rc = bn_fin_apply(z, cw.partials, g.ppg, count, *bn, d->eps, tr, st, d->has_res ? res : nullptr, y, d->N, d->Cout,
-                           g.HoWo, d->bn_groups, d->relu, s))) return rc;
-    if (!tr) return MEDT_OK;
-    if (Queue* q = queue_for(s)) {
-        q->fin.push_back(FinJob{make_fin(cw.partials, g.ppg, d->Cout, count, *bn, st), d->bn_groups, 2, d->momentum, d->eps});
-        return MEDT_OK;
-    }
-    return bn_finalize(cw.partials, g.ppg, d->bn_groups, d->Cout, count, *bn, d->momentum, d->eps, 2, st, s);
+    const bool bn1x1 = da->has_bn && db->has_bn && da->K == 1 && db->K == 1 && da->N == db->N;
+    if (bn1x1 && conv_small_ok(*da) && conv_small_ok(*db) && conv_small_pair_ok(*da, *db)) {
+        if ((rc = a.check_bn()) || (rc = b.check_bn())) return rc;
+        if ((rc = conv_small_fwd_pair(*da, xa, wa, *bna, resa, za, ya, a.partials, *db, xb, wb, *bnb, resb, zb, yb, b.partials, s)))
+            return rc;
+        if ((rc = a.finish_small(s))) return rc;
+        return b.finish_small(s);
+    }
+    if (bn1x1 && !conv_small_ok(*da) && !conv_small_ok(*db) &&
+        conv1x1_fwd_plain(da->N, da->bn_groups, da->Cin, da->H, da->W, da->Cout, da->K, da->stride, da->pad) &&
+        conv1x1_fwd_plain(db->N, db->bn_groups, db->Cin, db->H, db->W, db->Cout, db->K, db->stride, db->pad)) {
+        if ((rc = a.check_bn()) || (rc = b.check_bn())) return rc;
+        const Conv1x1Problem pa{xa, wa, za, a.tr ? a.partials : nullptr, da->N, da->Cin, da->H, da->W, da->Cout, da->stride, da->bn_groups};
+        const Conv1x1Problem pb{xb, wb, zb, b.tr ? b.partials : nullptr, db->N, db->Cin, db->H, db->W, db->Cout, db->stride, db->bn_groups};
+        if ((rc = conv1x1_fwd_pair(pa, pb, s))) return rc;
+        if ((rc = bn_fin_apply_pair(a.apply_problem(), b.apply_problem(), s))) return rc;
+        if ((rc = a.finish_generic(s))) return rc;
+        return b.finish_generic(s);
+    }
+    if ((rc = a.run(s))) return rc;
+    return b.run(s);
 }
 
 int medt_conv_block_bwd(const medt_conv_desc* d, const float* x, const float* w, const medt_bn_ptrs* bn, const float* z,
diff --git a/medical-transformer_amd/csrc/medt_kernels.h b/medical-transformer_amd/csrc/medt_kernels.h
--- a/medical-transformer_amd/csrc/medt_kernels.h
+++ b/medical-transformer_amd/csrc/medt_kernels.h
@@ -202,6 +202,27 @@
 int bn_fin_apply(const float* z, const float* partials, int ppg, double count, const medt_bn_ptrs& bn, float eps, int training,
                  BnStats st, const float* res, float* y, int N, int C, int HW, int groups, int relu, hipStream_t s);
 bool conv_fwd_ws_ok(int Cin, int Cout, int K, int stride, long positions);
+struct BnFinApplyProblem {
+    const float *z, *partials, *res;
+    const medt_bn_ptrs* bn;
+    float* y;
+    BnStats st;
+    int ppg, N, C, HW, groups, relu, training;
+    double count;
+    float eps;
+};
+int bn_fin_apply_pair(const BnFinApplyProblem& a, const BnFinApplyProblem& b, hipStream_t s);
+struct Conv1x1Problem {
+    const float *x, *w;
+    float *y, *partials;
+    int N, Cin, H, W, Cout, stride, groups;
+};
+bool conv1x1_fwd_plain(int N, int groups, int Cin, int H, int W, int Cout, int K, int stride, int pad);
+int conv1x1_fwd_pair(const Conv1x1Problem& a, const Conv1x1Problem& b, hipStream_t s);
+bool conv_small_pair_ok(const medt_conv_desc& a, const medt_conv_desc& b);
+int conv_small_fwd_pair(const medt_conv_desc& da, const float* xa, const float* wa, const medt_bn_ptrs& bna, const float* resa,
+                        float* za, float* ya, float* partialsa, const medt_conv_desc& db, const float* xb, const float* wb,
+                        const medt_bn_ptrs& bnb, const float* resb, float* zb, float* yb, float* partialsb, hipStream_t s);
 int bn_chan_threads(const medt_conv_desc& d, int HoWo);
 int bn_act_bwd_chan(const medt_conv_desc& d, const float* dy, const float* y, const float* z, BnStats st,
                     const float* weight, float* g, float* dz, float* partials, int HoWo, hipStream_t s);
diff --git a/medical-transformer_amd/medt_amd/_lib.py b/medical-transformer_amd/medt_amd/_lib.py
--- a/medical-transformer_amd/medt_amd/_lib.py
+++ b/medical-transformer_amd/medt_amd/_lib.py
@@ -117,6 +117,9 @@
     "medt_conv_workspace_bytes": (C.c_size_t, [C.POINTER(ConvDesc)]),
     "medt_conv_block_fwd": (C.c_int, [C.POINTER(ConvDesc), C.c_void_p, C.c_void_p, C.c_void_p, C.POINTER(BnPtrs),
                                       C.c_void_p, C.c_void_p, C.c_void_p, C.c_void_p, C.c_void_p, C.c_size_t, C.c_void_p]),
+    "medt_conv_block_pair_fwd": (C.c_int, [C.POINTER(ConvDesc), C.c_void_p, C.c_void_p, C.c_void_p, C.POINTER(BnPtrs),
+                                           C.c_void_p, C.c_void_p, C.c_void_p, C.c_void_p, C.c_void_p, C.c_size_t] * 2
+                                 + [C.c_void_p]),
     "medt_conv_block_bwd": (C.c_int, [C.POINTER(ConvDesc), C.c_void_p, C.c_void_p, C.POINTER(BnPtrs), C.c_void_p,
                                       C.c_void_p, C.c_void_p, C.c_void_p, C.c_void_p, C.c_void_p, C.c_void_p, C.c_void_p,
                                       C.c_void_p, C.c_void_p, C.c_void_p, C.c_void_p, C.c_size_t, C.c_void_p]),
diff --git a/medical-transformer_amd/medt_amd/net.py b/medical-transformer_amd/medt_amd/net.py
--- a/medical-transformer_amd/medt_amd/net.py
+++ b/medical-transformer_amd/medt_amd/net.py
@@ -14,6 +14,7 @@
 TWO_STREAMS = os.environ.get("MEDT_TWO_STREAMS", "1") != "0"
 SINKS = os.environ.get("MEDT_GRAD_SINKS", "1") != "0"
 EARLY_FIN = os.environ.get("MEDT_EARLY_FIN", "1") != "0"
+PAIR = os.environ.get("MEDT_PAIR", "1") != "0"
 _side = {}
 
 
@@ -47,6 +48,10 @@
     if pre is None:
         pre = {"down": None, "h": None, "w": None, "up": None}
     pre.setdefault("ds", None)
+    if PAIR and blk.downsample is not None and pre["down"] is None and pre["ds"] is None:
+        both = ops.conv_block_pair_pre(x, blk.conv_down, blk.bn1, True, blk.downsample[0], blk.downsample[1], False, bn_groups)
+        if both is not None:
+            pre["down"], pre["ds"] = both
     out = ops.conv_block(x, blk.conv_down, blk.bn1, relu=True, training=blk.bn1.training, bn_groups=bn_groups,
                          x_sink=sink, x_role="final", pre=pre["down"])
     out = blk.hight_block.run(out, bn_groups, False, pre["h"])
diff --git a/medical-transformer_amd/medt_amd/ops.py b/medical-transformer_amd/medt_amd/ops.py
--- a/medical-transformer_amd/medt_amd/ops.py
+++ b/medical-transformer_amd/medt_amd/ops.py
@@ -176,6 +176,46 @@
         training = torch.is_grad_enabled() and (x.requires_grad or conv.weight.requires_grad)
     return ConvBlockFn.apply(x, conv.weight, conv.bias, bn.weight if bn is not None else None,
                              bn.bias if bn is not None else None, res, cfg, training)
+
+
+PAIR_CALLS = 0
+
+
+def conv_block_pair_pre(x, conv_a, bn_a, relu_a, conv_b, bn_b, relu_b, bn_groups=1):
+    global PAIR_CALLS
+    if bn_a is None or bn_b is None or conv_a.bias is not None or conv_b.bias is not None:
+        return None
+    if conv_a.weight.shape[2] != 1 or conv_b.weight.shape[2] != 1:
+        return None
+    _require_device(x)
+    lib = L.lib()
+    x = x.contiguous()
+    N, _, H, W = x.shape
+    dev = x.device
+    args, outs, held = [], [], []
+    for conv, bn, relu in ((conv_a, bn_a, relu_a), (conv_b, bn_b, relu_b)):
+        cfg = ConvBlockCfg(conv.stride[0], conv.padding[0], bn, relu, bn_groups)
+        w = conv.weight
+        desc = _conv_desc(x, w, cfg, False, False, bn.training)
+        s, p = cfg.stride, cfg.pad
+        y = torch.empty((N, w.shape[0], (H + 2 * p - 1) // s + 1, (W + 2 * p - 1) // s + 1), device=dev, dtype=torch.float32)
+        z = torch.empty_like(y)
+        stats = torch.empty((max(lib.medt_conv_stats_floats(C.byref(desc)), 1),), device=dev, dtype=torch.float32)
+        ws_bytes = lib.medt_conv_workspace_bytes(C.byref(desc))
+        if ws_bytes == 0:
+            raise L.MedtError("conv block pair: " + lib.medt_last_error().decode())
+        ws = torch.empty((ws_bytes,), device=dev, dtype=torch.uint8)
+        bnp = _bn_ptrs(bn, bn.training)
+        held += [desc, bnp, ws, stats]
+        args += [C.byref(desc), x.data_ptr(), w.data_ptr(), None, C.byref(bnp), None, z.data_ptr(), y.data_ptr(),
+                 stats.data_ptr(), ws.data_ptr(), ws_bytes]
+        outs.append((z, y, stats))
+    q = DEFER.recording()
+    L.check(lib.medt_conv_block_pair_fwd(*args, _stream()), "medt_conv_block_pair_fwd")
+    PAIR_CALLS += 1
+    if q is not None:
+        q.hold(*(t for t in held if isinstance(t, torch.Tensor)))
+    return outs[0], outs[1]
 
 
 class UpReluAddFn(torch.autograd.Function):
```

Measured after the change: 2193 images/s (median of 6 runs). 1.5% higher.
